# maria-korosteleva/Garment-Pattern-Estimation

Measured on AMD Instinct MI355X. Metric: garments/sec (fwd+bwd) at N=2048 pts, batch 32 per GPU, higher is better.
Workload: dtype f16x3 (fp16 MFMA x3 per product, fp32 accumulate); 1 GPU; BASELINE cfg 2 (cfg 3 per GPU): GarmentFullPattern3D, EdgeConv encoder + LSTM decoders, N=2048, batch 32/GPU, k=16; fp32 storage, fp32-grade arithmetic: edge-GEMM products as 3 fp16 MFMAs on tensor-normalised two-term splits, fp32 accumulate (parity-grade: the exact mode's test bars); global_batch=32, parallelism=dp1, math_mode=f16x3, loss_epoch=0, reserved_cus=0, launch=eager (one Python call per launch), side_stream=True, step=fwd + ComposedPatternLoss + bwd + fused Adam (flat arena)

## Files before the change

garment-pattern-estimation_amd/_lib.py:

```python
import ctypes
import os
import re

import torch

_HERE = os.path.dirname(os.path.abspath(__file__))
LIB_PATH = os.environ.get('GPE_HIP_LIB') or os.path.join(_HERE, 'libgpe_hip.so')
HEADER_PATH = os.path.join(os.path.dirname(_HERE), 'include', 'gpe_hip.h')
EXT_HEADER_PATH = os.path.join(os.path.dirname(_HERE), 'include', 'gpe_hip_ext.h')
HEADERS = (HEADER_PATH, EXT_HEADER_PATH)
FIT_HEADER_PATH = os.path.join(os.path.dirname(_HERE), 'include', 'gpe_hip_fit.h')
FEATURE_HEADERS = (FIT_HEADER_PATH,)
EVAL_HEADER_PATH = os.path.join(os.path.dirname(_HERE), 'include', 'gpe_hip_eval.h')
EVAL_HEADERS = (EVAL_HEADER_PATH,)
PLACE_HEADER_PATH = os.path.join(os.path.dirname(_HERE), 'include', 'gpe_hip_place.h')
PLACE_HEADERS = (PLACE_HEADER_PATH,)
FRAMEWORK_HEADER_PATH = os.path.join(os.path.dirname(_HERE), 'include', 'gpe_hip_framework.h')
FRAMEWORK_HEADERS = (FRAMEWORK_HEADER_PATH,)

_CT = {'p': ctypes.c_void_p, 'i': ctypes.c_int, 'l': ctypes.c_long, 'f': ctypes.c_float, 'd': ctypes.c_double}


def _code(ctype):
    t = ctype.strip()
    if '*' in t:
        return 'p'
    t = t.replace('const', '').strip()
    return {'int': 'i', 'long': 'l', 'float': 'f', 'double': 'd'}[t]


def parse_header(path=HEADER_PATH):
    src = open(path).read()
    src = re.sub(r'/\*.*?\*/', ' ', src, flags=re.S)
    src = re.sub(r'//[^\n]*', ' ', src)
    sigs = {}
    for m in re.finditer(r'\b(int|long)\s+(gpe_\w+)\s*\(([^)]*)\)\s*;', src):
        res, name, args = m.group(1), m.group(2), m.group(3).strip()
        codes = []
        if args and args != 'void':
            for a in args.split(','):
                a = a.strip()
                ctype = a[:a.rfind(' ')] if '*' not in a else a[:a.rfind('*') + 1]
                codes.append(_code(ctype))
        sigs[name] = (_code(res), codes)
    unbound = sorted(set(re.findall(r'\b(gpe_\w+)\s*\(', src)) - set(sigs))
    if unbound:
        raise ValueError('%s: cannot bind the declaration of %s (only functions returning int or long are parsed)'
                         % (path, ', '.join(unbound)))
    return sigs


_lib = None


def lib():
    global _lib
    if _lib is None:
        if not os.path.exists(LIB_PATH):
            raise RuntimeError(
                'libgpe_hip.so not built: run `python -c "import __graft_entry__ as g; g.build()"` '
                '(hipcc --offload-arch=gfx950).  There is no CPU fallback for the product path.')
        l = ctypes.CDLL(LIB_PATH)
        for header in HEADERS + FEATURE_HEADERS + EVAL_HEADERS + PLACE_HEADERS + FRAMEWORK_HEADERS:
            for name, (res, args) in parse_header(header).items():
                fn = getattr(l, name)
                fn.restype = _CT[res]
                fn.argtypes = [_CT[a] for a in args]
        _lib = l
        env = os.environ.get('GPE_MATH')
        if env:
            set_math(env)
        dbg = os.environ.get('GPE_DEBUG_SET')
        if dbg:
            l.gpe_debug_set(int(dbg, 0))
    return _lib


MATH_MODES = {'f32': 0, 'bf16x3': 1, 'mixed': 2, 'bf16x6': 3, 'f16x3': 4}


def set_math(mode):
    if mode not in MATH_MODES:
        raise ValueError('unknown math mode %r (choose from %s)' % (mode, sorted(MATH_MODES)))
    prev = lib().gpe_math_set(MATH_MODES[mode])
    if prev < 0:
        raise RuntimeError('gpe_math_set failed with code %d' % prev)
    return {v: k for k, v in MATH_MODES.items()}[prev]


def set_f16x3_min_rows(rows):
    prev = lib().gpe_f16x3_min_rows_set(int(rows))
    if prev < 0:
        raise RuntimeError('gpe_f16x3_min_rows_set failed with code %d' % prev)
    return prev


def set_reserved_cus(n):
    prev = lib().gpe_reserve_cus_set(int(n))
    if prev < 0:
        raise ValueError('reserved CUs must lie in 0 .. 192')
    return prev


def get_reserved_cus():
    n = lib().gpe_reserve_cus_set(0)
    lib().gpe_reserve_cus_set(n)
    return n


def get_math():
    return {v: k for k, v in MATH_MODES.items()}[lib().gpe_math_get()]


def _conv(a):
    if a is None:
        return None
    if isinstance(a, torch.Tensor):
        return a.data_ptr()
    return a


TIMING = None


_raw_stream = getattr(torch._C, '_cuda_getCurrentRawStream', None)
_cur_device = getattr(torch._C, '_cuda_getDevice', None) or torch.cuda.current_device
_FN = {}


def call(name, *args):
    fn = _FN.get(name)
    if fn is None:
        fn = _FN[name] = getattr(lib(), name)
    cur = _cur_device()
    for a in args:
        if isinstance(a, torch.Tensor):
            if not a.is_cuda or a.device.index != cur:
                raise RuntimeError('%s: tensor on %s but the current device is cuda:%d — wrap the call in '
                                   'torch.cuda.device(...) (one process per GPU is the supported layout)'
                                   % (name, a.device, cur))
            break
    if TIMING is not None or _raw_stream is None:
        stream = torch.cuda.current_stream()
        handle = stream.cuda_stream
    else:
        handle = _raw_stream(cur)
# ... 14 lines not shown
```

garment-pattern-estimation_amd/_opbase.py:

```python
import torch

from . import _lib as L
from . import streams


F32 = torch.float32
F64 = torch.float64


def _dev_check(t):
    if not t.is_cuda:
        raise RuntimeError('gpe ops need tensors on the MI355X (got a %s tensor); there is no CPU path' % t.device)
    if t.dtype != F32:
        raise RuntimeError('gpe ops are fp32 (got %s)' % t.dtype)


def _rows2d(t):
    assert t.dim() == 2 and (t.shape[1] == 1 or t.stride(1) == 1), (t.shape, t.stride())
    return (t, t.stride(0), 0, 0)


def _rows3d(t):
    assert t.dim() == 3 and (t.shape[2] == 1 or t.stride(2) == 1), (t.shape, t.stride())
    return (t, t.stride(0), t.stride(1), t.shape[1])


def round_up(a, b):
    return (a + b - 1) // b * b


_WS = {}


def _workspace(nbytes, device):
    key = streams.stream_key(device)
    buf = _WS.get(key)
    if buf is None or buf.numel() < nbytes:
        buf = torch.empty(max(int(nbytes), 1 << 20), device=torch.device('cuda', key[0]), dtype=torch.uint8)
        _WS[key] = buf
    return buf


_EDGE_WS_BYTES = {}


def edge_workspace(B, N, k, ldmax, device):
    key = (B, N, k, ldmax)
    n = _EDGE_WS_BYTES.get(key)
    if n is None:
        n = L.query('gpe_edge_ws_bytes', B, N, k, ldmax)
        if n < 0:
            raise RuntimeError('gpe_edge_ws_bytes failed with code %d' % n)
        _EDGE_WS_BYTES[key] = n
    return _workspace(n, device), n


def f16x3_words(n, rows, device):
    if L.get_math() != 'f16x3' or rows < L.query('gpe_f16x3_min_rows'):
        return None
    return torch.zeros(n, device=device, dtype=torch.int32)


def _word(words, i):
    return None if words is None else words[i:i + 1]


_TICKETS = {}


def _ticket(device):
    key = streams.stream_key(device)
    t = _TICKETS.get(key)
    if t is None:
        t = _TICKETS[key] = torch.zeros(1, device=torch.device('cuda', key[0]), dtype=torch.int32)
    return t


def _stitch_ldw(H):
    nb = (H + 15) // 16
    nb = 4 if nb <= 4 else 8 if nb <= 8 else 13 if nb <= 13 else 16
    return nb * 16 if (nb * 16) % 32 == 16 else nb * 16 + 16


def _view_strides(ol):
    assert ol.dim() == 4 and ol.stride(3) == 1, (ol.shape, ol.stride())
    return ol.stride(0), ol.stride(1), ol.stride(2)


def _row_stride(t, P):
    assert t.dim() == 3 and t.stride(2) == 1 and t.stride(0) == P * t.stride(1), (t.shape, t.stride())
    return t.stride(1)


def _int_tensor(t, shape, name, dev):
    if (not torch.is_tensor(t) or tuple(t.shape) != shape or t.is_floating_point() or t.is_complex() or t.dtype == torch.bool
            or t.device != dev):
        raise ValueError('%s must be an integer %s tensor on the device of edges3d' % (name, list(shape)))


def _int32(t, lo, hi):
    t = t.detach()
    if t.dtype != torch.int32:
        t = t.to(torch.int64).clamp(lo, hi).to(torch.int32)
    return t.contiguous()
```

garment-pattern-estimation_amd/build.py:

```python
import concurrent.futures
import os
import subprocess
import sys

HERE = os.path.dirname(os.path.abspath(__file__))
CSRC = os.path.join(HERE, 'csrc')
OUT = os.path.join(HERE, 'libgpe_hip.so')
HIPCC = os.environ.get('HIPCC', '/opt/rocm/bin/hipcc')
FLAGS = ['--offload-arch=gfx950', '-O3', '-std=c++17', '-fPIC', '-Wall', '-Wno-unused-function',
         '-Wno-unused-variable', '-Wno-unused-but-set-variable']
EXTRA_FLAGS = {'gpe_edgegemm_sr_dense.hip': ['-mllvm', '-amdgpu-sched-strategy=max-ilp'],
               'gpe_redgemm.hip': ['-mllvm', '-amdgpu-sched-strategy=max-memory-clause'],
               'gpe_knn.hip': ['-mllvm', '-amdgpu-sched-strategy=max-ilp'],
               'gpe_knn_ft.hip': (['-DKNN_FT_TIMING'] if os.environ.get('KNN_FT_TIMING') else []) + os.environ.get('KNN_FT_FLAGS', '').split(),
               'gpe_edgegemm_x6.hip': ['-mllvm', '-amdgpu-sched-strategy=max-memory-clause'],
               'gpe_edgegemm_h3.hip': ['-mllvm', '-amdgpu-sched-strategy=max-ilp'],
               'gpe_edgegemm_w8_f3.hip': ['-mllvm', '-amdgpu-sched-strategy=max-ilp'],
               'gpe_edgegemm_w8_b3.hip': ['-mllvm', '-amdgpu-sched-strategy=max-ilp']}


def _sources():
    return sorted(f for f in os.listdir(CSRC) if f.endswith('.hip'))


def _stale(obj, src):
    if not os.path.exists(obj):
        return True
    t = os.path.getmtime(obj)
    inc = os.path.join(os.path.dirname(HERE), 'include')
    deps = [os.path.join(CSRC, src), os.path.abspath(__file__)]
    deps += [os.path.join(inc, h) for h in ('gpe_hip.h', 'gpe_hip_ext.h', 'gpe_hip_fit.h', 'gpe_hip_eval.h', 'gpe_hip_place.h',
                                              'gpe_hip_framework.h')]
    deps += [os.path.join(CSRC, h) for h in os.listdir(CSRC) if h.endswith('.h')]
    return any(os.path.getmtime(d) > t for d in deps)


COMPILED, REUSED = [], []


def _compile(src):
    obj = os.path.join(CSRC, src[:-4] + '.o')
    if not _stale(obj, src):
        REUSED.append(src)
    else:
        COMPILED.append(src)
        cmd = [HIPCC] + FLAGS + EXTRA_FLAGS.get(src, []) + ['-c', os.path.join(CSRC, src), '-o', obj]
        r = subprocess.run(cmd, capture_output=True, text=True)
        if r.returncode != 0:
            raise RuntimeError('hipcc failed on %s:\n%s' % (src, r.stderr[-6000:]))
        if r.stderr.strip():
            sys.stderr.write(r.stderr[-3000:])
    return obj


def build(force=False, verbose=True):
    force = force or os.environ.get('GPE_FORCE_BUILD') == '1'
    del COMPILED[:], REUSED[:]
    srcs = _sources()
    if force:
        for s in srcs:
            o = os.path.join(CSRC, s[:-4] + '.o')
            if os.path.exists(o):
                os.remove(o)
    with concurrent.futures.ThreadPoolExecutor(max_workers=min(8, len(srcs))) as ex:
        objs = list(ex.map(_compile, srcs))
    if (not os.path.exists(OUT)) or any(os.path.getmtime(o) > os.path.getmtime(OUT) for o in objs):
        cmd = [HIPCC, '--offload-arch=gfx950', '-shared', '-fPIC', '-o', OUT] + objs
        r = subprocess.run(cmd, capture_output=True, text=True)
        if r.returncode != 0:
            raise RuntimeError('link failed:\n' + r.stderr[-4000:])
        if verbose:
            print('built', OUT)
    if verbose:
        print('build: compiled %d source(s) %s; reused %d up-to-date object(s) %s (force=%s; GPE_FORCE_BUILD=1 or '
              'build(force=True) recompiles everything)' % (len(COMPILED), COMPILED, len(REUSED), REUSED, force))
    return OUT


if __name__ == '__main__':
    build(force='--force' in sys.argv)
```

garment-pattern-estimation_amd/csrc/gpe_common.h:

```cpp
#pragma once
#include <cstdlib>
#include <hip/hip_runtime.h>
#include <stdint.h>
#include "../../include/gpe_hip.h"
#include "../../include/gpe_hip_ext.h"
#include "../../include/gpe_hip_fit.h"
#include "../../include/gpe_hip_eval.h"
#include "../../include/gpe_hip_place.h"
#include "../../include/gpe_hip_framework.h"

#define GPE_OK 0
#define GPE_EINVAL (-22)
#define GPE_ELAUNCH (-5)

#define GPE_CHECK_LAUNCH()                                   \
    do {                                                     \
        hipError_t e_ = hipGetLastError();                   \
        if (e_ != hipSuccess) return GPE_ELAUNCH;            \
    } while (0)

typedef float f32x4 __attribute__((ext_vector_type(4)));

static inline bool gpe_overlap(const void* p, size_t n, const void* q, size_t m)
{
    if (!p || !q || !n || !m) return false;
    const uintptr_t a = (uintptr_t)p, b = (uintptr_t)q;
    return a < b + m && b < a + n;
}

static inline const char* gpe_dbg_env_str(const char* name)
{
    static const int on = getenv("GPE_DEBUG") ? atoi(getenv("GPE_DEBUG")) : 0;
    return on ? getenv(name) : nullptr;
}
static inline int gpe_dbg_env(const char* name, int dflt)
{
    const char* e = gpe_dbg_env_str(name);
    return e ? atoi(e) : dflt;
}

static inline int gpe_cdiv(long a, long b) { return (int)((a + b - 1) / b); }
static inline int gpe_round_up(int a, int b) { return (a + b - 1) / b * b; }

struct GpeRows {
    const float* base;
    long stride_outer;
    long stride_inner;
    int inner;
};

__device__ __forceinline__ const float* gpe_row_ptr(const GpeRows& a, long r)
{
    if (a.inner <= 0) return a.base + r * a.stride_outer;
    long o = r / a.inner;
    long i = r - o * a.inner;
    return a.base + o * a.stride_outer + i * a.stride_inner;
}

__device__ __forceinline__ bool gpe_aligned16(const void* p) { return (((uintptr_t)p) & 15) == 0; }

__device__ __forceinline__ unsigned gpe_udiv(unsigned n, unsigned d, double rcp)
{
    unsigned q = (unsigned)__double2uint_rz((double)n * rcp);
    const unsigned up = ((unsigned long long)(q + 1) * d <= n) ? 1u : 0u;
    const unsigned dn = ((unsigned long long)q * d > n) ? 1u : 0u;
    return q + up - dn;
}

#define GPE_ENSURE_MAX_LDS_N(fn, bytes_)                                                                         \
    do {                                                                                                         \
        static unsigned long long done_ = 0;                                                                     \
        int dev_ = 0;                                                                                            \
        if (hipGetDevice(&dev_) != hipSuccess) return GPE_ELAUNCH;                                               \
        const unsigned long long bit_ = 1ull << (dev_ & 63);                                                     \
        if (!(done_ & bit_)) {                                                                                   \
            if (hipFuncSetAttribute(reinterpret_cast<const void*>(fn), hipFuncAttributeMaxDynamicSharedMemorySize, \
                                    (bytes_)) != hipSuccess)                                                     \
                return GPE_ELAUNCH;                                                                              \
            done_ |= bit_;                                                                                       \
        }                                                                                                        \
    } while (0)

#define GPE_ENSURE_MAX_LDS(fn) GPE_ENSURE_MAX_LDS_N(fn, 160 * 1024)

int gpe_num_cus();
int gpe_math_rowgemm();
int gpe_math_redgemm();
#define GPE_WS_DUMMY_BYTES (64 * 512 * 4)
#define GPE_WS_H3_PARTS 1024
#define GPE_WS_H3_BYTES (((2 + 2 * GPE_WS_H3_PARTS) * 4 + 255) & ~255)
struct GpeEdgeWs { float* dummy; unsigned* h3; char* pseudo; size_t pseudo_bytes; };
static inline GpeEdgeWs gpe_edge_ws(void* ws, long bytes)
// ... 90 lines not shown
```

garment-pattern-estimation_amd/csrc/gpe_device.h:

```cpp
#pragma once
#include "gpe_common.h"
#include <math.h>

typedef _Float16 gpe_f16x2 __attribute__((ext_vector_type(2)));
typedef _Float16 gpe_f16x8 __attribute__((ext_vector_type(8)));
typedef __bf16 gpe_bf16x2 __attribute__((ext_vector_type(2)));
typedef __bf16 gpe_bf16x8 __attribute__((ext_vector_type(8)));
typedef float gpe_f32x2 __attribute__((ext_vector_type(2)));
typedef unsigned gpe_u32x2 __attribute__((ext_vector_type(2)));
typedef unsigned gpe_u32x4 __attribute__((ext_vector_type(4)));

__device__ __forceinline__ float gpe_sigmoid(float x) { return 1.f / (1.f + expf(-x)); }

__device__ __forceinline__ void gpe_split2_f16(float a, float b, unsigned& h, unsigned& l)
{
    const gpe_f32x2 v = {a, b};
    const gpe_f16x2 hh = __builtin_convertvector(v, gpe_f16x2);
    const gpe_f32x2 r = v - __builtin_convertvector(hh, gpe_f32x2);
    h = __builtin_bit_cast(unsigned, hh);
    l = __builtin_bit_cast(unsigned, __builtin_convertvector(r, gpe_f16x2));
}
__device__ __forceinline__ void gpe_split2_f16(float a, float b, float s, unsigned& h, unsigned& l) { gpe_split2_f16(a * s, b * s, h, l); }

__device__ __forceinline__ unsigned gpe_cvt2_bf16(float a, float b)
{
    const gpe_f32x2 v = {a, b};
    return __builtin_bit_cast(unsigned, __builtin_convertvector(v, gpe_bf16x2));
}
__device__ __forceinline__ void gpe_split2_bf16(float a, float b, unsigned& h, unsigned& l)
{
    h = gpe_cvt2_bf16(a, b);
    l = gpe_cvt2_bf16(a - __uint_as_float(h << 16), b - __uint_as_float(h & 0xffff0000u));
}

#define GPE_STATE_SA 4096.f
#define GPE_STATE_INV_SA (1.f / 4096.f)

__device__ __forceinline__ gpe_u32x4 gpe_philox4x32(unsigned c0, unsigned c1, unsigned c2, unsigned c3, unsigned k0, unsigned k1)
{
#pragma unroll
    for (int r = 0; r < 10; ++r) {
        const unsigned hi0 = __umulhi(0xD2511F53u, c0), lo0 = 0xD2511F53u * c0;
        const unsigned hi1 = __umulhi(0xCD9E8D57u, c2), lo1 = 0xCD9E8D57u * c2;
        c0 = hi1 ^ c1 ^ k0; c1 = lo1; c2 = hi0 ^ c3 ^ k1; c3 = lo0;
        k0 += 0x9E3779B9u; k1 += 0xBB67AE85u;
    }
    return gpe_u32x4{c0, c1, c2, c3};
}
struct gpe_rng {
    unsigned k0, k1, d0, d1, b8;
    __device__ __forceinline__ gpe_u32x4 operator()(int kind, unsigned item, unsigned attempt = 0) const
    {
        return gpe_philox4x32(item | ((unsigned)kind << 28), attempt | b8, d0, d1, k0, k1);
    }
};

#define GPE_SPIN_LIMIT (1u << 23)

__device__ __forceinline__ unsigned gpe_flag_load(const unsigned* flag)
{
    return __hip_atomic_load(flag, __ATOMIC_RELAXED, __HIP_MEMORY_SCOPE_AGENT);
}
__device__ __forceinline__ unsigned gpe_flag_poll(const unsigned* flag) { return __builtin_amdgcn_readfirstlane(gpe_flag_load(flag)); }
__device__ __forceinline__ void gpe_flag_wait(const unsigned* flag, unsigned need)
{
    unsigned spins = 0;
    while (gpe_flag_poll(flag) < need) {
        __builtin_amdgcn_s_sleep(1);
        if (++spins > GPE_SPIN_LIMIT) __builtin_trap();
    }
    asm volatile("" ::: "memory");
}
__device__ __forceinline__ void gpe_drain_stores() { asm volatile("s_waitcnt vmcnt(0)" ::: "memory"); }
__device__ __forceinline__ unsigned gpe_flag_ticket(unsigned* flag)
{
    return __hip_atomic_fetch_add(flag, 1u, __ATOMIC_RELAXED, __HIP_MEMORY_SCOPE_AGENT);
}
__device__ __forceinline__ void gpe_flag_arrive_wave(unsigned* flag)
{
    gpe_drain_stores();
    if ((threadIdx.x & 63) == 0) gpe_flag_ticket(flag);
}
__device__ __forceinline__ void gpe_flag_arrive_wg(unsigned* flag, unsigned long long* stamp = nullptr)
{
    gpe_drain_stores();
    if (stamp && threadIdx.x == 0) *stamp = wall_clock64();
    __syncthreads();
// ... 50 lines not shown
```

garment-pattern-estimation_amd/csrc/gpe_edgegemm_h3.hip:

```cpp
#include "gpe_edgegemm_split_kernel.h"

#define H3_PQ_BLOCKS GPE_WS_H3_PARTS

__global__ __launch_bounds__(256) void gpe_h3_absmax_kernel(const float* __restrict__ x, long rows, int cols4, long ld,
                                                            unsigned* __restrict__ out)
{
    const long total = rows * cols4;
    unsigned m = 0u;
    for (long t = (long)blockIdx.x * blockDim.x + threadIdx.x; t < total; t += (long)gridDim.x * blockDim.x) {
        const long r = t / cols4;
        const int q = (int)(t - r * cols4);
        const float4 v = ld4(x + r * ld + 4 * q);
        const unsigned a = __float_as_uint(v.x) & 0x7fffffffu, b = __float_as_uint(v.y) & 0x7fffffffu;
        const unsigned c = __float_as_uint(v.z) & 0x7fffffffu, d = __float_as_uint(v.w) & 0x7fffffffu;
        const unsigned ab = a > b ? a : b, cd = c > d ? c : d;
        const unsigned e = ab > cd ? ab : cd;
        m = m > e ? m : e;
    }
#pragma unroll
    for (int o = 32; o > 0; o >>= 1) {
        const unsigned t = (unsigned)__shfl_xor((int)m, o);
        m = m > t ? m : t;
    }
    __shared__ unsigned red[4];
    if ((threadIdx.x & 63) == 0) red[threadIdx.x >> 6] = m;
    __syncthreads();
    if (threadIdx.x == 0) {
        const unsigned a = red[0] > red[1] ? red[0] : red[1], b = red[2] > red[3] ? red[2] : red[3];
        const unsigned r = a > b ? a : b;
        if (r) atomicMax(out, r);
    }
}

__global__ __launch_bounds__(256) void gpe_h3_pqmax_kernel(const float* __restrict__ pq, long rows, int H, long ld,
                                                           float* __restrict__ part )
{
    const int lane = threadIdx.x & 63, wave = threadIdx.x >> 6;
    const int h4 = H >> 2;
    float mp = -INFINITY, mq = -INFINITY;
    const long stride = (long)gridDim.x * 4;
    for (long r = (long)blockIdx.x * 4 + wave; r < rows; r += 2 * stride) {
        const float* row0 = pq + r * ld;
        const bool two = r + stride < rows;
        const float* row1 = pq + (two ? r + stride : r) * ld;
        for (int q = lane; q < 2 * h4; q += 64) {
            const float4 v0 = ld4(row0 + 4 * q), v1 = ld4(row1 + 4 * q);
            const float m = fmaxf(fmaxf(fmaxf(v0.x, v0.y), fmaxf(v0.z, v0.w)), fmaxf(fmaxf(v1.x, v1.y), fmaxf(v1.z, v1.w)));
            if (q < h4) mp = fmaxf(mp, m); else mq = fmaxf(mq, m);
        }
    }
#pragma unroll
    for (int o = 32; o > 0; o >>= 1) { mp = fmaxf(mp, __shfl_xor(mp, o)); mq = fmaxf(mq, __shfl_xor(mq, o)); }
    __shared__ float red[8];
    if (lane == 0) { red[2 * wave] = mp; red[2 * wave + 1] = mq; }
    __syncthreads();
    if (threadIdx.x == 0) {
        part[2 * blockIdx.x] = fmaxf(fmaxf(red[0], red[2]), fmaxf(red[4], red[6]));
        part[2 * blockIdx.x + 1] = fmaxf(fmaxf(red[1], red[3]), fmaxf(red[5], red[7]));
    }
}

__global__ __launch_bounds__(1024) void gpe_h3_wmax_kernel(const float* __restrict__ w, long n, unsigned* __restrict__ slots,
                                                           unsigned* __restrict__ clear_word)
{
    __shared__ unsigned red[16];
    unsigned m = 0u;
    for (long t = threadIdx.x; t < n; t += 1024) {
        const unsigned a = __float_as_uint(w[t]) & 0x7fffffffu;
        m = m > a ? m : a;
    }
#pragma unroll
    for (int o = 32; o > 0; o >>= 1) {
        const unsigned t = (unsigned)__shfl_xor((int)m, o);
        m = m > t ? m : t;
    }
    if ((threadIdx.x & 63) == 0) red[threadIdx.x >> 6] = m;
    __syncthreads();
    if (threadIdx.x == 0) {
        for (int i = 1; i < 16; ++i) m = m > red[i] ? m : red[i];
        slots[1] = m;
        slots[0] = 0u;
        if (clear_word) clear_word[0] = 0u;
    }
}

__global__ __launch_bounds__(256) void gpe_h3_pqfinish_kernel(const float* __restrict__ part, int nblk, unsigned* __restrict__ slots)
{
    float mp = -INFINITY, mq = -INFINITY;
    for (int b = threadIdx.x; b < nblk; b += 256) { mp = fmaxf(mp, part[2 * b]); mq = fmaxf(mq, part[2 * b + 1]); }
#pragma unroll
    for (int o = 32; o > 0; o >>= 1) { mp = fmaxf(mp, __shfl_xor(mp, o)); mq = fmaxf(mq, __shfl_xor(mq, o)); }
    __shared__ float red[8];
    if ((threadIdx.x & 63) == 0) { red[2 * (threadIdx.x >> 6)] = mp; red[2 * (threadIdx.x >> 6) + 1] = mq; }
    __syncthreads();
    if (threadIdx.x == 0) {
        mp = fmaxf(fmaxf(red[0], red[2]), fmaxf(red[4], red[6]));
        mq = fmaxf(fmaxf(red[1], red[3]), fmaxf(red[5], red[7]));
        float b = (mp + mq) * 1.000001f;
        if (!(b > 0.f)) b = (b != b) ? b : 0.f;
        slots[0] = __float_as_uint(b) & 0x7fffffffu;
    }
}

int gpe_h3_pq_passes(unsigned* out, float* part, const float* pq, long rows, int H, long ld, hipStream_t s)
{
    if (!out || !part || (H & 3)) return GPE_EINVAL;
    int gx = (int)((rows + 3) / 4);
    if (gx > H3_PQ_BLOCKS) gx = H3_PQ_BLOCKS;
    hipLaunchKernelGGL(gpe_h3_pqmax_kernel, dim3(gx), dim3(256), 0, s, pq, rows, H, ld, part);
    GPE_CHECK_LAUNCH();
    hipLaunchKernelGGL(gpe_h3_pqfinish_kernel, dim3(1), dim3(256), 0, s, part, gx, out);
    GPE_CHECK_LAUNCH();
    return GPE_OK;
}
static int h3_absmax_pass(unsigned* out, const float* x, long rows, int cols4, long ld, hipStream_t s)
{
    int gx = (int)((rows * cols4 + 255) / 256);
    const int cap = gpe_num_cus() * 8;
    if (gx > cap) gx = cap;
    hipLaunchKernelGGL(gpe_h3_absmax_kernel, dim3(gx), dim3(256), 0, s, x, rows, cols4, ld, out);
    GPE_CHECK_LAUNCH();
    return GPE_OK;
}
int gpe_h3_absmax(unsigned* out, const float* x, long rows, int cols, long ld, hipStream_t s)
{
    if (!out || !x) return GPE_EINVAL;
    if (hipMemsetAsync(out, 0, sizeof(unsigned), s) != hipSuccess) return GPE_ELAUNCH;
    const int cols4 = (cols + 3) >> 2;
    if (rows * cols4 <= 0) return GPE_OK;
    return h3_absmax_pass(out, x, rows, cols4, ld, s);
}

int gpe_edge_f16x3_scales(RgParams& p, long npts, int amode, int emode, int KCH, hipStream_t s)
{
    unsigned* slots = p.ws.h3;
    const bool tracks = emode == E_EDGE_FWD || emode == E_BWD_INPLACE;
    const bool reuse = (p.dbg & 128) != 0;
    const long wn = (long)16 * KCH * p.Npad;
    const bool w_ready = p.w_ready && p.user_amax_a;
    if (!reuse && !w_ready) {
        hipLaunchKernelGGL(gpe_h3_wmax_kernel, dim3(1), dim3(1024), 0, s, p.wp, wn, slots, tracks ? p.user_amax_out : nullptr);
        GPE_CHECK_LAUNCH();
    }
    p.h3_amax_a = (p.user_amax_a && !reuse) ? p.user_amax_a : slots;
    if (!p.user_amax_a && !reuse) {
        const int rc = amode == A_DENSE ? h3_absmax_pass(slots, p.a.base, p.M, (p.K + 3) >> 2, (long)p.a.stride_outer, s)
                                        : gpe_h3_pq_passes(slots, reinterpret_cast<float*>(slots + 2), p.pq, npts, p.H, (long)p.ldpq, s);
        if (rc != GPE_OK) return rc;
    }
    p.h3_amax_w = slots + 1;
// ... 11 lines not shown
```

garment-pattern-estimation_amd/csrc/gpe_knn.hip:

```cpp
#include "gpe_device.h"
#include "gpe_knn_plan.h"
#include <math.h>
#include <stdint.h>
#include <stdlib.h>

#define KNN_CCH 32
#define KNN_LD 36
#define KNN_LDD 68

__device__ __forceinline__ float knn_readlane_f(float v, int l)
{
    return __int_as_float(__builtin_amdgcn_readlane(__float_as_int(v), l));
}

__device__ __forceinline__ float knn_sub(float a, float b)
{
    float d;
    asm("v_sub_f32 %0, %1, %2" : "=v"(d) : "v"(a), "v"(b));
    return d;
}
__device__ __forceinline__ float knn_sqacc(float d, float acc)
{
    asm("v_fma_f32 %0, %1, %1, %0" : "+v"(acc) : "v"(d));
    return acc;
// ... 584 lines not shown
        asm volatile("s_waitcnt lgkmcnt(0)" ::: "memory");

        const int cand = c0 + lane;
#pragma unroll
        for (int i = 0; i < 16; ++i) {
            if (!((qm >> i) & 1u)) continue;
            const float d = dW[i * KNN_LDD + lane];
            float ldv = ld_[i];
            int liv = li_[i];
            const float t = knn_select_mf(c0 == c_first, d, lane, cand, K2, kk, knn_readlane_f(m2e_of, i),
                                          knn_readlane_f(thrq, i), mW, ldv, liv);
            ld_[i] = ldv; li_[i] = liv;
            thrq = ((lane & 15) == i) ? t : thrq;
            __builtin_amdgcn_sched_barrier(0);
        }
    }
#pragma unroll
    for (int i = 0; i < 16; ++i) {
        const int q = q0 + 16 * wave + i;
        if (q < N && lane < K2)
            part[(((size_t)b * N + q) * nsplit + piece) * K2 + lane] =
                ((unsigned long long)(unsigned)__float_as_int(ld_[i]) << 32) | (unsigned)li_[i];
    }
}

#define KNN_H3_CCH 64
#define KNN_H3_PITCH 160

__global__ __launch_bounds__(256) void gpe_knn_planes_kernel(const float* __restrict__ x, long rows, int C, int ldx, int CP,
                                                             _Float16* __restrict__ pl, float* __restrict__ isc,
                                                             const int* __restrict__ order, int N)
{
    const int lane = threadIdx.x & 63;
    const long r0 = ((long)blockIdx.x * 4 + (threadIdx.x >> 6)) * KNN_NORM_ROWS;
    if (r0 >= rows) return;
    const long last = rows - 1;
    long src[KNN_NORM_ROWS];
#pragma unroll
    for (int u = 0; u < KNN_NORM_ROWS; ++u) {
        const long r = (r0 + u < last) ? r0 + u : last;
        src[u] = order ? (r / N) * N + order[r] : r;
    }
    float m[KNN_NORM_ROWS];
#pragma unroll
    for (int u = 0; u < KNN_NORM_ROWS; ++u) m[u] = 0.f;
    for (int c0 = 0; c0 < C; c0 += 64) {
        const int c = c0 + lane;
        const int cc = (c < C) ? c : 0;
        float v[KNN_NORM_ROWS];
#pragma unroll
        for (int u = 0; u < KNN_NORM_ROWS; ++u) v[u] = x[src[u] * ldx + cc];
#pragma unroll
        for (int u = 0; u < KNN_NORM_ROWS; ++u) m[u] = (c < C) ? fmaxf(m[u], fabsf(v[u])) : m[u];
    }
    float sc[KNN_NORM_ROWS];
#pragma unroll
    for (int u = 0; u < KNN_NORM_ROWS; ++u) {
        float t = m[u];
#pragma unroll
        for (int o = 32; o > 0; o >>= 1) t = fmaxf(t, __int_as_float(__builtin_amdgcn_ds_bpermute((lane ^ o) << 2, __float_as_int(t))));
        float s_, inv_;
        gpe_h3_scale_of(__float_as_uint(t), s_, inv_);
        sc[u] = s_;
        if (lane == 0 && r0 + u <= last) isc[r0 + u] = inv_;
    }
    for (int c0 = 0; c0 < CP; c0 += 64) {
        const int c = c0 + lane;
        if (c >= CP) break;
        const int cc = (c < C) ? c : 0;
        float v[KNN_NORM_ROWS];
#pragma unroll
        for (int u = 0; u < KNN_NORM_ROWS; ++u) v[u] = x[src[u] * ldx + cc];
#pragma unroll
        for (int u = 0; u < KNN_NORM_ROWS; ++u) {
            if (r0 + u <= last) {
                const float xs = (c < C) ? v[u] * sc[u] : 0.f;
                const _Float16 h = (_Float16)xs;
                const _Float16 l = (_Float16)(xs - (float)h);
                _Float16* row = pl + (r0 + u) * 2 * (long)CP;
                row[c] = h;
                row[CP + c] = l;
            }
        }
    }
}

template <int NBMAX>
__global__ __launch_bounds__(256, 2) void gpe_knn_h3_kernel(const _Float16* __restrict__ pl, const float* __restrict__ isc, int N,
                                                            int CP, int kk, int K2, const float* __restrict__ norms,
                                                            const int* __restrict__ cmax, float ce, int B, int tiles, int pin,
                                                            int nsplit, unsigned long long* __restrict__ part, int probe,
                                                            const int* __restrict__ ord)
{
    const int rot = ord != nullptr;
    extern __shared__ __align__(16) float smem[];
    constexpr int PLANE_B = KNN_TC * KNN_H3_PITCH;
    constexpr int BUF_B = 2 * PLANE_B;
    char* const cB = reinterpret_cast<char*>(smem);
    float* const dS = reinterpret_cast<float*>(cB + 2 * BUF_B);
    unsigned long long* const mS = reinterpret_cast<unsigned long long*>(dS + 4 * 16 * KNN_LDD);
    float* const npS = reinterpret_cast<float*>(mS + 4 * 64);
    float* const isS = npS + 2 * KNN_TC;

    const int tid = threadIdx.x;
    const int lane = tid & 63;
    const int wave = __builtin_amdgcn_readfirstlane(tid >> 6);
    int b, item;
    const int ipc = tiles * nsplit;
    if (pin) {
        const int xcd = blockIdx.x & (GPE_NXCD - 1), slot = blockIdx.x >> 3;
        const int jc = slot / ipc;
        b = xcd + GPE_NXCD * jc;
        item = slot - jc * ipc;
        if (b >= B) return;
    } else {
        b = blockIdx.x / ipc;
        item = blockIdx.x - b * ipc;
    }
    const int qt = item / nsplit, piece = item - qt * nsplit;
    const int q0 = qt * KNN_TQ;
    const int tps = (tiles + nsplit - 1) / nsplit;
    const int c_first = piece * tps * KNN_TC;
    const int c_stop = ((piece + 1) * tps * KNN_TC < N) ? (piece + 1) * tps * KNN_TC : N;
    const _Float16* cloud = pl + (size_t)b * N * 2 * CP;
    const float* cnorm = norms + (size_t)b * N;
    const float* cisc = isc + (size_t)b * N;
    const int* cord = ord ? ord + (size_t)b * N : nullptr;
    auto pt = [&](int r) -> int { return cord ? cord[r] : r; };
    float* const dW = dS + wave * 16 * KNN_LDD;
    unsigned long long* const mW = mS + wave * 64;

    float ld_[16];
    int li_[16];
#pragma unroll
    for (int i = 0; i < 16; ++i) { ld_[i] = INFINITY; li_[i] = -1; }
    float thrq = INFINITY;

    const int j = lane & 15, g = lane >> 4;
    const int myq = (q0 + 16 * wave + j < N) ? q0 + 16 * wave + j : N - 1;
    const float nq = cnorm[pt(myq)];
    const float fq = -2.f * cisc[myq];
    const float cm = __int_as_float(cmax[b]);
    float m2e_of;
    {
        const int qi = (q0 + 16 * wave + (lane & 15) < N) ? q0 + 16 * wave + (lane & 15) : N - 1;
        m2e_of = 2.02f * ce * (cnorm[pt(qi)] + cm);
    }
    const int NB = CP >> 5;
    gpe_u32x4 qh[NBMAX], ql[NBMAX];
    {
        const _Float16* qrow = cloud + (size_t)myq * 2 * CP;
#pragma unroll
        for (int blk = 0; blk < NBMAX; ++blk) {
            const int bb = (blk < NB) ? blk : 0;
            qh[blk] = *reinterpret_cast<const gpe_u32x4*>(qrow + 32 * bb + 8 * g);
            ql[blk] = *reinterpret_cast<const gpe_u32x4*>(qrow + CP + 32 * bb + 8 * g);
        }
    }
    const int nchunk = (CP + KNN_H3_CCH - 1) / KNN_H3_CCH;
    gpe_u32x4 pre[4];
    float pre_n = 0.f, pre_s = 0.f;
    int pre_first = 0, pre_tp = 0;
    const int ntile_p = (c_stop - c_first + KNN_TC - 1) / KNN_TC;
    int v_start = 0;
    if (rot && ntile_p > 0) {
        v_start = qt - 1 - c_first / KNN_TC;
// ... 290 lines not shown

__global__ __launch_bounds__(256) void gpe_knn_rerank2_kernel(const float* __restrict__ x, long nq_total, int N, int C, int ldx, int k,
                                                              const unsigned long long* __restrict__ part,
                                                              const float* __restrict__ norms, const int* __restrict__ cmax,
                                                              float ce, int32_t* __restrict__ idx, int32_t* __restrict__ idx_glob)
{
    __shared__ unsigned long long strip[4][64];
    const int lane = threadIdx.x & 63;
    const int wave = __builtin_amdgcn_readfirstlane(threadIdx.x >> 6);
    const long q0 = ((long)blockIdx.x * 4 + wave) * 2;
    if (q0 >= nq_total) return;
    unsigned long long* const mW = strip[wave];
    const int h = lane >> 5, l = lane & 31;
    const bool two = q0 + 1 < nq_total;
    const long q = (h && two) ? q0 + 1 : q0;
    unsigned long long key = part[q * 64 + l];
    const unsigned long long hi32 = part[q * 64 + 32 + l];
    const unsigned long long v_lo = __ballot(key != ~0ull), v_hi = __ballot(hi32 != ~0ull);
    const bool packable = (v_hi == 0ull) && k <= 32;
    if (!packable) {
        knn_rerank_query(x, q0, N, C, ldx, k, 64, 1, part, norms, cmax, ce, idx, idx_glob, 1, mW);
        if (two) knn_rerank_query(x, q0 + 1, N, C, ldx, k, 64, 1, part, norms, cmax, ce, idx, idx_glob, 1, mW);
        return;
    }
    const int nv = __builtin_popcount((unsigned)(v_lo >> (32 * h)));
    const int nvmax = max(__builtin_popcount((unsigned)v_lo), __builtin_popcount((unsigned)(v_lo >> 32)));
    const int base = 32 * h;
    {
        int rank = 0;
        const int klo = (int)(unsigned)key, khi = (int)(unsigned)(key >> 32);
        for (int s2 = 0; s2 < nvmax; ++s2) {
            const unsigned long long kn = ((unsigned long long)(unsigned)__shfl(khi, base + s2) << 32) | (unsigned)__shfl(klo, base + s2);
            rank += (s2 < nv && (kn < key || (kn == key && s2 < l))) ? 1 : 0;
        }
        if (l >= nv) rank = l;
        mW[base + rank] = key;
        asm volatile("s_waitcnt lgkmcnt(0)" ::: "memory");
        key = mW[lane];
        asm volatile("s_waitcnt lgkmcnt(0)" ::: "memory");
    }
    const float da = __int_as_float((int)(key >> 32));
    const int id = (int)(unsigned)key;
    const int b = (int)(q / N);
    const float* cloud = x + (size_t)b * N * ldx;
    const float* qrow = x + q * ldx;
    const bool vec4 = (ldx % 4 == 0) && ((uintptr_t)x % 16 == 0);
    const float m2e = 2.02f * ce * (norms[q] + __int_as_float(cmax[b]));
    const float T = __shfl(da, base + k - 1) + m2e;
    const unsigned long long below = __ballot(l < nv && da <= T);
    const int m = __builtin_popcount((unsigned)(below >> base));
    const int mmax = max(__builtin_popcount((unsigned)below), __builtin_popcount((unsigned)(below >> 32)));
    const bool in_s = l < m;
    const float dnext = __shfl(da, (lane + 1) & 63);
    const bool near_next = (l + 1 < m) && (dnext - da <= m2e);
    const unsigned long long nn = __ballot(near_next);
    const bool near_prev = (l > 0) && ((nn >> (lane - 1)) & 1ull);
    const bool flagged = in_s && (near_next || near_prev);
    const unsigned long long fl = __ballot(flagged);
    int newpos = l;
    if (fl) {
        const unsigned long long starts = __ballot(in_s && !near_prev);
        const unsigned long long le = ((lane == 63) ? ~0ull : ((1ull << (lane + 1)) - 1ull)) & (0xffffffffull << base);
        const int start = 63 - __builtin_clzll((starts & le) | (1ull << base));
        float dex = da;
        if (flagged) dex = knn_exact_chain(qrow, cloud + (size_t)id * ldx, C, vec4);
        int r = 0;
        for (int s2 = 0; s2 < mmax; ++s2) {
            const float dj = __shfl(dex, base + s2);
            const int ij = __shfl(id, base + s2);
            const int sj = __shfl(start, base + s2);
            r += (s2 < m && sj == start && (dj < dex || (dj == dex && ij < id))) ? 1 : 0;
        }
        if (flagged) newpos = (start - base) + r;
    }
    if (in_s && newpos < k && (h == 0 || two)) {
        idx[q * k + newpos] = id;
        if (idx_glob) idx_glob[q * k + newpos] = b * N + id;
    }
}

int gpe_knn_launch_prologue(const GpeKnnCall& c, const GpeKnnPlan& p)
{
    const long nq = (long)c.B * c.N;
    if (p.identity) {
        hipLaunchKernelGGL(gpe_knn_identity_order_kernel, dim3((unsigned)gpe_cdiv(nq, 256)), dim3(256), 0, c.stream, c.order_out, nq, c.N);
        GPE_CHECK_LAUNCH();
    }
    if (p.norms) {
        hipLaunchKernelGGL(gpe_knn_norms_kernel, dim3((unsigned)gpe_cdiv(nq, 4 * KNN_NORM_ROWS)), dim3(256), 0, c.stream, c.x, nq, c.N, c.C,
                           c.ldx, p.norms, p.cmax);
        GPE_CHECK_LAUNCH();
        hipLaunchKernelGGL(gpe_knn_cmax_kernel, dim3(c.B), dim3(256), 0, c.stream, p.norms, c.N, p.cmax);
        GPE_CHECK_LAUNCH();
    }
    if (p.planes) {
        hipLaunchKernelGGL(gpe_knn_planes_kernel, dim3((unsigned)gpe_cdiv(nq, 4 * KNN_NORM_ROWS)), dim3(256), 0, c.stream, c.x, nq, c.C,
                           c.ldx, p.CP, p.planes, p.iscale, p.order, c.N);
        GPE_CHECK_LAUNCH();
    }
    return GPE_OK;
}

int gpe_knn_launch_lists(const GpeKnnCall& c, const GpeKnnPlan& p)
{
    const size_t lds = (size_t)2 * 2 * KNN_TC * KNN_H3_PITCH + (size_t)4 * 16 * KNN_LDD * sizeof(float) +
                       4 * 64 * sizeof(unsigned long long) + 4 * KNN_TC * sizeof(float);
    auto go = [&](auto kernel) {
        hipLaunchKernelGGL(kernel, dim3((unsigned)p.nblocks), dim3(256), lds, c.stream, p.planes, p.iscale, c.N, p.CP, c.k, p.K2, p.norms,
                           p.cmax, p.ce, c.B, p.tiles, p.pin, p.nsplit, p.part, p.probe, p.order);
    };
    if (p.NB <= 2) go(gpe_knn_h3_kernel<2>);
    else if (p.NB <= 5) go(gpe_knn_h3_kernel<5>);
    else go(gpe_knn_h3_kernel<8>);
    GPE_CHECK_LAUNCH();
    return GPE_OK;
}

int gpe_knn_launch_f32filter(const GpeKnnCall& c, const GpeKnnPlan& p)
{
    const size_t lds = ((size_t)2 * KNN_TQ * KNN_MF_LD + 4 * 16 * KNN_LDD) * sizeof(float) + 4 * 64 * sizeof(unsigned long long) +
                       KNN_TC * sizeof(float);
    auto go = [&](auto kernel) {
        hipLaunchKernelGGL(kernel, dim3((unsigned)p.nblocks), dim3(256), lds, c.stream, c.x, c.N, c.C, c.ldx, c.k, p.K2, p.norms, p.cmax,
                           p.ce, c.B, p.tiles, p.pin, p.nsplit, p.part, p.probe);
    };
    if (p.vec == 4) go(gpe_knn_mfma_kernel<4>);
    else if (p.vec == 2) go(gpe_knn_mfma_kernel<2>);
    else go(gpe_knn_mfma_kernel<1>);
    GPE_CHECK_LAUNCH();
    return GPE_OK;
}

int gpe_knn_launch_recheck(const GpeKnnCall& c, const GpeKnnPlan& p)
{
    const long nq = (long)c.B * c.N;
    if (p.rerank2)
        hipLaunchKernelGGL(gpe_knn_rerank2_kernel, dim3((unsigned)gpe_cdiv(nq, 8)), dim3(256), 0, c.stream, c.x, nq, c.N, c.C, c.ldx, c.k,
                           p.part, p.norms, p.cmax, p.ce, c.idx, c.idx_glob);
    else
        hipLaunchKernelGGL(gpe_knn_rerank_kernel, dim3((unsigned)gpe_cdiv(nq, 4)), dim3(256), 0, c.stream, c.x, nq, c.N, c.C, c.ldx, c.k,
                           p.K2, p.nsplit, p.part, p.norms, p.cmax, p.ce, c.idx, c.idx_glob, p.unsorted);
    GPE_CHECK_LAUNCH();
    return GPE_OK;
}
```

garment-pattern-estimation_amd/csrc/gpe_knn_plan.h:

```cpp
#pragma once
#include "gpe_common.h"

#define KNN_TQ 64
#define KNN_TC 64
#define KNN_MF_MINC 16
#define KNN_H3_MAXC 256
#define KNN_FT_NBMAX 5
#define KNN_FT_MAXK 32
#define KNN_FT_CAP 64
#define K3_MINN 128
#define K3_MAXN 8192
#ifndef K3_QW
#define K3_QW 4
#endif
#define KNN_FILTER_MAXK 48

struct GpeKnnSwitches {
    int PROBE;
    int PIN;
    int VEC;
    int SPLIT;
    int EXACT;
    int F32FILTER;
    int SORTED;
    int NOORDER;
    int FT;
    int RR2;
};
const GpeKnnSwitches& gpe_knn_switches();

struct GpeKnnCall {
    const float* x; int B, N, C, ldx, k;
    int32_t* idx; int32_t* idx_glob;
    const int32_t* order_in; int32_t* order_out;
    void* ws; long ws_bytes;
    hipStream_t stream;
};

static_assert(sizeof(float4) + 8 * sizeof(float) <= 64 * sizeof(unsigned long long), "sorted cloud + tile boxes must fit the list region");
struct GpeKnnWs {
    size_t lists_bytes;
    size_t norms, cmax, planes, iscale;
    size_t tb, sorted_bytes;
    size_t need_f32;
    size_t need_h3;
    size_t total;
};
static inline size_t gpe_knn_up256(size_t b) { return (b + 255) & ~(size_t)255; }
static inline GpeKnnWs gpe_knn_ws_layout(int B, int N, int C)
{
    GpeKnnWs w;
    const size_t nq = (size_t)B * N;
    const size_t norm_bytes = gpe_knn_up256(nq * sizeof(float)), cmax_bytes = gpe_knn_up256((size_t)B * sizeof(int));
    const size_t CP = ((size_t)C + 31) & ~(size_t)31;
    const size_t pl_bytes = gpe_knn_up256(nq * 2 * CP * sizeof(_Float16));
    w.lists_bytes = nq * 64 * sizeof(unsigned long long);
    w.norms = w.lists_bytes;
    w.cmax = w.norms + norm_bytes;
    w.planes = w.cmax + cmax_bytes;
    w.iscale = w.planes + pl_bytes;
    w.tb = nq * sizeof(float4);
    w.sorted_bytes = w.tb + (size_t)B * gpe_cdiv(N, 64) * 8 * sizeof(float);
    w.need_f32 = w.planes + 256;
    w.need_h3 = w.need_f32 + pl_bytes + norm_bytes;
    w.total = ((C >= KNN_MF_MINC && C <= KNN_H3_MAXC) ? w.need_h3 : w.need_f32) + 256;
    return w;
}
static inline size_t gpe_knn_split_bytes(int B, int N, int nsplit, int k) { return (size_t)B * N * nsplit * k * sizeof(unsigned long long); }

enum GpeKnnPath {
    GPE_KNN_NOTHING,
    GPE_KNN_SORTED3,
    GPE_KNN_ALLPAIRS,
    GPE_KNN_SCAN,
    GPE_KNN_LISTS,
    GPE_KNN_F32FILTER
};
struct GpeKnnPlan {
    GpeKnnPath path; int rc;
    bool identity;
    int pin, tiles, nsplit, vec;
    long nblocks;
    int probe; bool smallc;
    int K2, CP, NB; float ce;
    bool wide; int qtiles;
    bool rerank2; int unsorted;
    const int32_t* order;
    unsigned long long* part;
    float* norms; int* cmax; _Float16* planes; float* iscale;
    float4* xs; float* tb;
};

static inline int gpe_knn_k2(int k, int N)
{
    int K2 = (2 * k < 32) ? 2 * k : 32;
    if (K2 < k + 8) K2 = k + 8;
    if (K2 > 64) K2 = 64;
    if (K2 > N) K2 = N;
    return K2;
}
static inline bool gpe_knn_valid(const GpeKnnCall& c)
{
    return c.x && c.idx && c.B >= 0 && c.N > 0 && c.C > 0 && c.ldx >= c.C && c.k > 0 && c.k <= 64 && c.k <= c.N &&
           (long)c.B * c.N * c.k < (1L << 31);
}
static inline bool gpe_knn_ws_holds(const GpeKnnCall& c, size_t bytes) { return c.ws && !(((uintptr_t)c.ws) & 15) && (size_t)c.ws_bytes >= bytes; }
static inline long gpe_knn_tile_blocks(int pin, int B, int tiles) { return pin ? (long)GPE_NXCD * gpe_cdiv(B, GPE_NXCD) * tiles : (long)B * tiles; }
static inline GpeKnnPlan gpe_knn_refuse(GpeKnnPlan p, int rc) { p.path = GPE_KNN_NOTHING; p.rc = rc; p.identity = false; return p; }

static inline GpeKnnPlan gpe_knn_plan_allpairs(GpeKnnPlan p, const GpeKnnCall& c, int usable_cus, const GpeKnnSwitches& sw, bool with_ws)
{
    p.path = GPE_KNN_ALLPAIRS;
    p.nsplit = 1;
    if (p.pin) {
        const double table = (double)c.N * c.ldx * sizeof(float), l2_budget = 3.2 * 1024 * 1024;
        const int resident = 4 * usable_cus / GPE_NXCD;
        for (;;) {
            const double clouds = (double)resident / ((double)p.tiles * p.nsplit);
            if (table * (clouds > 1.0 ? clouds : 1.0) <= l2_budget) break;
            if (clouds <= 1.0) break;
            if (p.nsplit >= 4 || 2 * p.nsplit * c.k > 64 || 2 * p.nsplit > p.tiles) break;
            p.nsplit *= 2;
        }
    }
    if (sw.SPLIT > 0 && sw.SPLIT * c.k <= 64 && sw.SPLIT <= p.tiles) p.nsplit = sw.SPLIT;
    if (p.nsplit > 1) {
        if (with_ws && gpe_knn_ws_holds(c, gpe_knn_split_bytes(c.B, c.N, p.nsplit, c.k))) p.part = (unsigned long long*)c.ws;
        else p.nsplit = 1;
    }
    p.nblocks = gpe_knn_tile_blocks(p.pin, c.B, p.tiles) * p.nsplit;
    if (p.nblocks >= (1L << 31)) return gpe_knn_refuse(p, GPE_EINVAL);
    const uintptr_t xa = (uintptr_t)c.x;
    p.vec = (c.C % 4 == 0 && c.ldx % 4 == 0 && xa % 16 == 0) ? 4 : (c.C % 2 == 0 && c.ldx % 2 == 0 && xa % 8 == 0) ? 2 : 1;
    if (sw.VEC > 0 && sw.VEC < p.vec) p.vec = sw.VEC;
    p.probe = sw.PROBE;
    p.smallc = !p.probe && p.vec == 1 && c.C <= 4;
    return p;
}

static inline GpeKnnPlan gpe_knn_plan(const GpeKnnCall& c, int usable_cus, const GpeKnnSwitches& sw)
{
    GpeKnnPlan p = {};
    p.path = GPE_KNN_NOTHING;
    p.rc = GPE_OK;
    if (!gpe_knn_valid(c)) return gpe_knn_refuse(p, GPE_EINVAL);
    if (c.B == 0) return p;
    p.tiles = gpe_cdiv(c.N, KNN_TQ);
    p.pin = (sw.PIN >= 0) ? (sw.PIN && c.B >= GPE_NXCD) : (gpe_pin_clouds(c.B) ? 1 : 0);
    p.nsplit = 1;
    const GpeKnnWs w = gpe_knn_ws_layout(c.B, c.N, c.C);
    if (c.C < KNN_MF_MINC || c.k > KNN_FILTER_MAXK || sw.EXACT) {
        if (c.C == 3 && sw.SORTED != 0 && c.N >= K3_MINN && c.N <= K3_MAXN && gpe_knn_ws_holds(c, w.sorted_bytes) &&
            (long)c.B * gpe_cdiv(c.N, 4 * K3_QW) < (1L << 31)) {
            p.path = GPE_KNN_SORTED3;
            p.tiles = gpe_cdiv(c.N, 64);
            p.qtiles = gpe_cdiv(c.N, 4 * K3_QW);
            p.nblocks = (long)c.B * p.qtiles;
            p.xs = reinterpret_cast<float4*>(c.ws);
            p.tb = reinterpret_cast<float*>(reinterpret_cast<char*>(c.ws) + w.tb);
            return p;
        }
        p.identity = c.order_out != nullptr;
        return gpe_knn_plan_allpairs(p, c, usable_cus, sw, true);
    }
    p.identity = c.order_out != nullptr;
    p.K2 = gpe_knn_k2(c.k, c.N);
    if (sw.SPLIT > 0 && sw.SPLIT * p.K2 <= 64 && sw.SPLIT <= p.tiles) p.nsplit = sw.SPLIT;
    bool h3 = !sw.F32FILTER && c.C <= KNN_H3_MAXC;
    if (h3 && (!c.ws || (size_t)c.ws_bytes < w.need_h3)) h3 = false;
    if (!gpe_knn_ws_holds(c, h3 ? w.need_h3 : w.need_f32)) return gpe_knn_plan_allpairs(p, c, usable_cus, sw, false);
    char* const scratch = (char*)c.ws;
    p.part = (unsigned long long*)scratch;
    p.norms = (float*)(scratch + w.norms);
    p.cmax = (int*)(scratch + w.cmax);
    p.CP = (c.C + 31) & ~31;
    p.NB = p.CP >> 5;
    p.ce = (6.f * c.C + (h3 ? 32.f : 16.f)) * 5.9604645e-8f;
    p.probe = sw.PROBE;
    p.nblocks = gpe_knn_tile_blocks(p.pin, c.B, p.tiles) * p.nsplit;
    if (p.nblocks >= (1L << 31)) return gpe_knn_refuse(p, GPE_EINVAL);
    if (!h3) {
        p.path = GPE_KNN_F32FILTER;
        const uintptr_t xa = (uintptr_t)c.x;
        p.vec = (c.ldx % 4 == 0 && xa % 16 == 0 && ((c.C + 3) & ~3) <= c.ldx) ? 4
              : (c.ldx % 2 == 0 && xa % 8 == 0 && ((c.C + 1) & ~1) <= c.ldx) ? 2 : 1;
        if (sw.VEC > 0 && sw.VEC < p.vec) p.vec = sw.VEC;
        return p;
    }
    p.planes = (_Float16*)(scratch + w.planes);
    p.iscale = (float*)(scratch + w.iscale);
    p.order = sw.NOORDER ? nullptr : c.order_in;
    if (sw.FT && p.NB <= KNN_FT_NBMAX && c.k <= KNN_FT_MAXK && p.nsplit == 1) {
        p.path = GPE_KNN_SCAN;
        p.wide = sw.FT == 8 || (sw.FT != 4 && (long)c.B * gpe_cdiv(c.N, 128) >= usable_cus);
        p.qtiles = gpe_cdiv(c.N, p.wide ? 128 : 64);
        p.nblocks = gpe_knn_tile_blocks(p.pin, c.B, p.qtiles);
        p.rerank2 = sw.RR2 != 0;
        p.unsorted = 1;
        return p;
    }
    p.path = GPE_KNN_LISTS;
    return p;
}

int gpe_knn_launch_prologue(const GpeKnnCall& c, const GpeKnnPlan& p);
int gpe_knn_launch_allpairs(const GpeKnnCall& c, const GpeKnnPlan& p);
int gpe_knn_launch_lists(const GpeKnnCall& c, const GpeKnnPlan& p);
int gpe_knn_launch_f32filter(const GpeKnnCall& c, const GpeKnnPlan& p);
int gpe_knn_launch_recheck(const GpeKnnCall& c, const GpeKnnPlan& p);
int gpe_knn_launch_sorted(const GpeKnnCall& c, const GpeKnnPlan& p);
int gpe_knn_launch_scan(const GpeKnnCall& c, const GpeKnnPlan& p);
```

garment-pattern-estimation_amd/csrc/gpe_knn_search.hip:

```cpp
#include "gpe_knn_plan.h"

const GpeKnnSwitches& gpe_knn_switches()
{
    static const GpeKnnSwitches sw = {gpe_dbg_env("GPE_KNN_PROBE", 0),  gpe_dbg_env("GPE_KNN_PIN", -1),  gpe_dbg_env("GPE_KNN_VEC", 0),
                                      gpe_dbg_env("GPE_KNN_SPLIT", 0),  gpe_dbg_env("GPE_KNN_EXACT", 0), gpe_dbg_env("GPE_KNN_F32FILTER", 0),
                                      gpe_dbg_env("GPE_KNN_SORTED", 1), gpe_dbg_env("GPE_KNN_NOORDER", 0), gpe_dbg_env("GPE_KNN_FT", 1),
                                      gpe_dbg_env("GPE_KNN_RR2", 1)};
    return sw;
}

extern "C" long gpe_knn_ws_bytes(int B, int N, int C, int k)
{
    if (B < 0 || N <= 0 || C <= 0 || k <= 0 || k > 64) return GPE_EINVAL;
    return (long)gpe_knn_ws_layout(B, N, C).total;
}

extern "C" int gpe_knn(const float* x, int B, int N, int C, int ldx, int k, int32_t* idx, int32_t* idx_glob, const int32_t* order_in,
                       int32_t* order_out, void* ws, long ws_bytes, void* stream)
{
    const GpeKnnCall c = {x, B, N, C, ldx, k, idx, idx_glob, order_in, order_out, ws, ws_bytes, (hipStream_t)stream};
    if (!gpe_knn_valid(c)) return GPE_EINVAL;
    const GpeKnnPlan p = gpe_knn_plan(c, B ? gpe_num_cus() : 0, gpe_knn_switches());
    if (p.path == GPE_KNN_NOTHING) return p.rc;
    int rc = gpe_knn_launch_prologue(c, p);
    if (rc != GPE_OK) return rc;
    switch (p.path) {
    case GPE_KNN_SORTED3: return gpe_knn_launch_sorted(c, p);
    case GPE_KNN_ALLPAIRS: return gpe_knn_launch_allpairs(c, p);
    case GPE_KNN_SCAN: rc = gpe_knn_launch_scan(c, p); break;
    case GPE_KNN_LISTS: rc = gpe_knn_launch_lists(c, p); break;
    default: rc = gpe_knn_launch_f32filter(c, p); break;
    }
    return rc != GPE_OK ? rc : gpe_knn_launch_recheck(c, p);
}
```

garment-pattern-estimation_amd/csrc/gpe_pointwise.hip:

```cpp
#include "gpe_device.h"
#include <math.h>

__device__ __forceinline__ float4 pw_ld4(const float* p) { return *reinterpret_cast<const float4*>(p); }
__device__ __forceinline__ void pw_st4(float* p, float4 v) { *reinterpret_cast<float4*>(p) = v; }

static int gpe_pack_kpad(int K)
{
    const int k16 = gpe_round_up(K, 16);
    return (k16 > 96 && k16 < 160) ? 160 : (k16 > 160 && k16 < 208) ? 208 : k16;
}
extern "C" long gpe_packed_size(int N, int K) { return (long)gpe_round_up(N, 16) * gpe_pack_kpad(K); }

__global__ void gpe_pack_kernel(const float* __restrict__ w, int ldw, int N, int K, int transpose,
                                const float* __restrict__ col_scale, float* __restrict__ wp, int Npad, long total)
{
    const long e = (long)blockIdx.x * blockDim.x + threadIdx.x;
    if (e >= total) return;
    const int t = (int)(e & 3);
    const long r = e >> 2;
    const int n = (int)(r % Npad);
    const long kq = r / Npad;
    const int k = (int)(kq * 4 + t);
    float v = 0.f;
    if (n < N && k < K) {
// ... 515 lines not shown
        s += __shfl_xor(s, o);
        q += __shfl_xor(q, o);
    }
    if (sub == 0) { red[wave][0][ch] = s; red[wave][1][ch] = q; }
    __syncthreads();
    if (wave != 0 || sub != 0 || c >= C) return;
    s = 0; q = 0;
    for (int w_ = 0; w_ < BNF_WAVES; ++w_) { s += red[w_][0][ch]; q += red[w_][1][ch]; }
    const double mean = s / count;
    double var = q / count - mean * mean;
    if (var < 0) var = 0;
    const double rstd = 1.0 / sqrt(var + (double)eps);
    const float sc = (float)((double)gamma[c] * rstd);
    stats[c] = (float)mean;
    stats[C + c] = (float)rstd;
    stats[2 * C + c] = sc;
    stats[3 * C + c] = (float)((double)beta[c] - mean * (double)sc);
    if (running_mean) {
        const double unbiased = (count > 1) ? var * count / (count - 1) : var;
        running_mean[c] = (float)((1.0 - momentum) * running_mean[c] + momentum * mean);
        running_var[c] = (float)((1.0 - momentum) * running_var[c] + momentum * unbiased);
    }
}

extern "C" int gpe_bn_finalize(const double* part, int nblk, int C, double count, const float* gamma,
                               const float* beta, float eps, float momentum, float* running_mean,
                               float* running_var, int64_t* num_batches, float* stats_out, void* stream)
{
    if (!part || !gamma || !beta || !stats_out || nblk <= 0 || C <= 0 || count <= 0) return GPE_EINVAL;
    hipLaunchKernelGGL(gpe_bn_finalize_kernel, dim3(gpe_cdiv(C, BNF_CPW)), dim3(64 * BNF_WAVES), 0, (hipStream_t)stream, part, nblk,
                       C, count, gamma, beta, eps, momentum, running_mean, running_var, num_batches, stats_out);
    GPE_CHECK_LAUNCH();
    return GPE_OK;
}

__global__ void gpe_bn_from_running_kernel(const float* rm, const float* rv, int C, const float* gamma,
                                           const float* beta, float eps, float* stats)
{
    const int c = blockIdx.x * blockDim.x + threadIdx.x;
    if (c >= C) return;
    const double rstd = 1.0 / sqrt((double)rv[c] + (double)eps);
    const float sc = (float)((double)gamma[c] * rstd);
    stats[c] = rm[c];
    stats[C + c] = (float)rstd;
    stats[2 * C + c] = sc;
    stats[3 * C + c] = (float)((double)beta[c] - (double)rm[c] * (double)sc);
}

extern "C" int gpe_bn_from_running(const float* running_mean, const float* running_var, int C, const float* gamma,
                                   const float* beta, float eps, float* stats_out, void* stream)
{
    if (!running_mean || !running_var || !gamma || !beta || !stats_out || C <= 0) return GPE_EINVAL;
    hipLaunchKernelGGL(gpe_bn_from_running_kernel, dim3(gpe_cdiv(C, 64)), dim3(64), 0, (hipStream_t)stream,
                       running_mean, running_var, C, gamma, beta, eps, stats_out);
    GPE_CHECK_LAUNCH();
    return GPE_OK;
}

__global__ void gpe_edge_finish_kernel(const float* __restrict__ mx, const float* __restrict__ mn, int ldagg,
                                       const float* __restrict__ stats, long rows, int C, float* __restrict__ y,
                                       int ldy)
{
    const long e = (long)blockIdx.x * blockDim.x + threadIdx.x;
    if (e >= rows * C) return;
    const long r = e / C;
    const int c = (int)(e - r * C);
    const float s = stats[2 * C + c], t = stats[3 * C + c];
    const float v = (s >= 0.f) ? mx[r * ldagg + c] : mn[r * ldagg + c];
    y[r * ldy + c] = s * v + t;
}

extern "C" int gpe_edge_finish(const float* mx, const float* mn, int ldagg, const float* stats, long rows, int C,
                               float* y, int ldy, void* stream)
{
    if (!mx || !mn || !stats || !y || rows < 0 || C <= 0 || ldagg < C || ldy < C) return GPE_EINVAL;
    if (rows == 0) return GPE_OK;
    hipLaunchKernelGGL(gpe_edge_finish_kernel, dim3(gpe_cdiv(rows * C, 256)), dim3(256), 0, (hipStream_t)stream, mx,
                       mn, ldagg, stats, rows, C, y, ldy);
    GPE_CHECK_LAUNCH();
    return GPE_OK;
}

#define PS_BLOCKS 512
__global__ __launch_bounds__(256) void gpe_point_sums_kernel(const float* __restrict__ g, int ldg,
                                                             const float* __restrict__ mx,
                                                             const float* __restrict__ mn, int ldagg,
                                                             const float* __restrict__ stats, long rows, int C,
                                                             double* __restrict__ part, unsigned* __restrict__ amax_sg)
{
    const int c = blockIdx.y * 256 + threadIdx.x;
    double s1 = 0, s2 = 0;
    float gm = 0.f, sabs = 0.f;
    if (c < C) {
        const float mean = stats[c], rstd = stats[C + c], s = stats[2 * C + c];
        const float* sp = (s >= 0.f) ? mx : mn;
        const long st = gridDim.x;
        long r = blockIdx.x;
        for (; r + 7 * st < rows; r += 8 * st) {
            float gv[8], sv[8];
#pragma unroll
            for (int u = 0; u < 8; ++u) { gv[u] = g[(r + u * st) * ldg + c]; sv[u] = sp[(r + u * st) * ldagg + c]; }
#pragma unroll
            for (int u = 0; u < 8; ++u) {
                s1 += (double)gv[u];
                s2 += (double)gv[u] * (double)((sv[u] - mean) * rstd);
                gm = fmaxf(gm, fabsf(gv[u]));
            }
        }
        for (; r < rows; r += st) {
            const float gv = g[r * ldg + c];
            const float sel = sp[r * ldagg + c];
            s1 += (double)gv;
            s2 += (double)gv * (double)((sel - mean) * rstd);
            gm = fmaxf(gm, fabsf(gv));
        }
        part[(size_t)blockIdx.x * 2 * C + c] = s1;
        part[(size_t)blockIdx.x * 2 * C + C + c] = s2;
        sabs = fabsf(s);
    }
    if (amax_sg) {
        float m = gm * sabs;
#pragma unroll
        for (int o = 32; o > 0; o >>= 1) m = fmaxf(m, __shfl_xor(m, o));
        if ((threadIdx.x & 63) == 0) atomicMax(amax_sg, __float_as_uint(m * 1.0000002f));
    }
}

extern "C" int gpe_point_sums_blocks(void) { return PS_BLOCKS; }

extern "C" int gpe_edge_bwd_point_sums(const float* g, int ldg, const float* mx, const float* mn, int ldagg,
                                       const float* stats, long rows, int C, double* part, uint32_t* amax_sg, void* stream)
{
    if (!g || !mx || !mn || !stats || !part || rows <= 0 || C <= 0) return GPE_EINVAL;
    if (amax_sg && hipMemsetAsync(amax_sg, 0, sizeof(uint32_t), (hipStream_t)stream) != hipSuccess) return GPE_ELAUNCH;
    hipLaunchKernelGGL(gpe_point_sums_kernel, dim3(PS_BLOCKS, gpe_cdiv(C, 256)), dim3(256), 0, (hipStream_t)stream, g, ldg, mx, mn,
                       ldagg, stats, rows, C, part, amax_sg);
    GPE_CHECK_LAUNCH();
    return GPE_OK;
}

#define BNC_WAVES 16
__global__ __launch_bounds__(64 * BNC_WAVES) void gpe_bn_bwd_coef_kernel(const double* __restrict__ part, int nblk,
                                                                        const float* __restrict__ stats, int C, double count,
                                                                        float* __restrict__ coef, float* dgamma, float* dbeta)
{
    __shared__ double red[BNC_WAVES][2][64];
    const int lane = threadIdx.x & 63, wave = threadIdx.x >> 6;
    const int c = blockIdx.x * 64 + lane;
    double s1 = 0, s2 = 0;
    if (c < C) {
        for (int b = wave; b < nblk; b += BNC_WAVES) {
            s1 += part[(size_t)b * 2 * C + c];
            s2 += part[(size_t)b * 2 * C + C + c];
        }
    }
    red[wave][0][lane] = s1;
    red[wave][1][lane] = s2;
    __syncthreads();
    if (wave != 0 || c >= C) return;
    s1 = 0; s2 = 0;
    for (int w_ = 0; w_ < BNC_WAVES; ++w_) { s1 += red[w_][0][lane]; s2 += red[w_][1][lane]; }
    const double mean = stats[c], rstd = stats[C + c], s = stats[2 * C + c];
    const double m1 = s1 / count, m2 = s2 / count;
    const double k2 = s * rstd * m2;
    coef[c] = (float)s;
    coef[C + c] = (float)(s * m1);
    coef[2 * C + c] = (float)k2;
    coef[3 * C + c] = (float)mean;
    if (dgamma) dgamma[c] = (float)s2;
    if (dbeta) dbeta[c] = (float)s1;
}

extern "C" int gpe_bn_bwd_coef(const double* part, int nblk, const float* stats, int C, double count, float* coef,
                               float* dgamma, float* dbeta, void* stream)
{
    if (!part || !stats || !coef || nblk <= 0 || C <= 0 || count <= 0) return GPE_EINVAL;
    hipLaunchKernelGGL(gpe_bn_bwd_coef_kernel, dim3(gpe_cdiv(C, 64)), dim3(64 * BNC_WAVES), 0, (hipStream_t)stream, part, nblk,
                       stats, C, count, coef, dgamma, dbeta);
    GPE_CHECK_LAUNCH();
    return GPE_OK;
}

#define DZ3_RB 8
__global__ __launch_bounds__(256) void gpe_dz3_kernel(float* __restrict__ a3, int lda3, const float* __restrict__ g,
                                                      int ldg, const uint8_t* __restrict__ amx,
                                                      const uint8_t* __restrict__ amn, int ldagg,
                                                      const float* __restrict__ coef, long npts, int k, int F,
                                                      float gscale, unsigned* __restrict__ amax_out)
{
    __shared__ unsigned amax_red[4];
    if (threadIdx.x < 4) amax_red[threadIdx.x] = 0u;
    __syncthreads();
    float amax_run = 0.f;
    const int lane = threadIdx.x & 63;
    const int wave = __builtin_amdgcn_readfirstlane(threadIdx.x >> 6);
    const int c = (blockIdx.y * 64 + lane) << 2;
    if (c >= F) return;
    const bool all_slots = amx == nullptr;
    float cs_[4], c1_[4], k2_[4], mu_[4];
#pragma unroll
    for (int t = 0; t < 4; ++t) {
        const int cc = (c + t < F) ? c + t : c;
        cs_[t] = coef[cc]; c1_[t] = coef[F + cc]; k2_[t] = coef[2 * F + cc]; mu_[t] = coef[3 * F + cc];
    }
    const long nw = (long)gridDim.x * 4;
    for (long i = (long)blockIdx.x * 4 + wave; i < npts; i += nw) {
        uint8_t mxv[4] = {0, 0, 0, 0}, mnv[4] = {0, 0, 0, 0};
        if (!all_slots) {
            const uchar4 smx = *reinterpret_cast<const uchar4*>(amx + i * ldagg + c);
            const uchar4 smn = *reinterpret_cast<const uchar4*>(amn + i * ldagg + c);
            mxv[0] = smx.x; mxv[1] = smx.y; mxv[2] = smx.z; mxv[3] = smx.w;
            mnv[0] = smn.x; mnv[1] = smn.y; mnv[2] = smn.z; mnv[3] = smn.w;
        }
        int sel[4];
        float sg[4];
#pragma unroll
        for (int t = 0; t < 4; ++t) {
            const int cc = (c + t < F) ? c + t : c;
            sel[t] = (cs_[t] >= 0.f) ? mxv[t] : mnv[t];
            sg[t] = cs_[t] * g[i * ldg + cc] * gscale;
        }
        float* base = a3 + i * k * lda3 + c;
        for (int s0 = 0; s0 < k; s0 += DZ3_RB) {
            float4 a[DZ3_RB];
#pragma unroll
            for (int u = 0; u < DZ3_RB; ++u) {
                const int s_ = (s0 + u < k) ? s0 + u : k - 1;
                a[u] = pw_ld4(base + (long)s_ * lda3);
            }
#pragma unroll
            for (int u = 0; u < DZ3_RB; ++u) {
                if (s0 + u < k) {
                    const float av[4] = {a[u].x, a[u].y, a[u].z, a[u].w};
                    float o[4];
#pragma unroll
                    for (int t = 0; t < 4; ++t) {
                        const float hit = (all_slots || sel[t] == s0 + u) ? sg[t] : 0.f;
                        o[t] = (c + t < F && av[t] > 0.f) ? hit - c1_[t] - (av[t] - mu_[t]) * k2_[t] : 0.f;
                    }
                    pw_st4(base + (long)(s0 + u) * lda3, make_float4(o[0], o[1], o[2], o[3]));
                    amax_run = fmaxf(fmaxf(amax_run, fmaxf(fabsf(o[0]), fabsf(o[1]))), fmaxf(fabsf(o[2]), fabsf(o[3])));
                }
            }
        }
    }
    if (amax_out) {
        atomicMax(&amax_red[wave], __float_as_uint(amax_run));
        __syncthreads();
        if (threadIdx.x == 0) {
            const unsigned a = amax_red[0] > amax_red[1] ? amax_red[0] : amax_red[1];
            const unsigned b = amax_red[2] > amax_red[3] ? amax_red[2] : amax_red[3];
            atomicMax(amax_out, a > b ? a : b);
        }
    }
}

static int dz3_launch(float* a3, int lda3, const float* g, int ldg, const uint8_t* amx, const uint8_t* amn, int ldagg,
                      const float* coef, int B, int N, int k, int F, float gscale, unsigned* amax_out, hipStream_t stream)
{
    if (!a3 || !g || !coef || B <= 0 || N <= 0 || k <= 0 || F <= 0 || (lda3 & 3) || lda3 < F) return GPE_EINVAL;
    if (amx && (!amn || (ldagg & 3) || ldagg < F)) return GPE_EINVAL;
    const long E = (long)B * N * k;
    if (E >= (1L << 31)) return GPE_EINVAL;
    const long npts = (long)B * N;
    const int blocks = (int)((npts + 3) / 4 < 4096 ? (npts + 3) / 4 : 4096);
    if (amax_out && hipMemsetAsync(amax_out, 0, sizeof(unsigned), stream) != hipSuccess) return GPE_ELAUNCH;
    hipLaunchKernelGGL(gpe_dz3_kernel, dim3(blocks, gpe_cdiv(F, 256)), dim3(256), 0, stream, a3, lda3, g, ldg, amx, amn,
                       ldagg, coef, npts, k, F, gscale, amax_out);
    GPE_CHECK_LAUNCH();
    return GPE_OK;
}

extern "C" int gpe_edge_dz3(float* a3, int lda3, const float* g, int ldg, const uint8_t* amx, const uint8_t* amn,
                            int ldagg, const float* coef, int B, int N, int k, int F, uint32_t* amax_out, void* stream)
{
    if (!amx || !amn) return GPE_EINVAL;
    return dz3_launch(a3, lda3, g, ldg, amx, amn, ldagg, coef, B, N, k, F, 1.f, amax_out, (hipStream_t)stream);
}

extern "C" int gpe_edge_dz3_all(float* a3, int lda3, const float* g, int ldg, float gscale, const float* coef, int B,
                                int N, int k, int F, uint32_t* amax_out, void* stream)
{
    return dz3_launch(a3, lda3, g, ldg, nullptr, nullptr, 0, coef, B, N, k, F, gscale, amax_out, (hipStream_t)stream);
}

#define BNG_FQ 16
__global__ __launch_bounds__(64 * BNG_FQ) void gpe_bn_bwd_from_G_kernel(
    const float* __restrict__ G, int ldG, const float* __restrict__ db, const float* __restrict__ w, int ldw, int Cn,
    int C, const float* __restrict__ stats, double* __restrict__ sums, float* __restrict__ dw, int lddw)
{
    __shared__ double red[BNG_FQ][2][64];
    const int lane = threadIdx.x & 63, fq = threadIdx.x >> 6;
    const int c = blockIdx.x * 64 + lane;
    double a = 0, b = 0;
    if (c < C) {
        const double s = stats[2 * C + c], t = stats[3 * C + c], mean = stats[c];
        const double beta = t + mean * s;
        double a2[2] = {0, 0}, b2[2] = {0, 0};
        int f = fq;
        for (; f + BNG_FQ < Cn; f += 2 * BNG_FQ) {
#pragma unroll
            for (int u = 0; u < 2; ++u) {
                const int ff = f + BNG_FQ * u;
                const double wf = w[(size_t)ff * ldw + c], gf = G[(size_t)ff * ldG + c], dbf = db[ff];
                a2[u] += wf * dbf;
                b2[u] += wf * gf;
                if (dw) dw[(size_t)ff * lddw + c] = (float)(gf * s + dbf * beta);
            }
        }
        if (f < Cn) {
            const double wf = w[(size_t)f * ldw + c], gf = G[(size_t)f * ldG + c], dbf = db[f];
            a2[0] += wf * dbf;
            b2[0] += wf * gf;
            if (dw) dw[(size_t)f * lddw + c] = (float)(gf * s + dbf * beta);
        }
        a = a2[0] + a2[1];
        b = b2[0] + b2[1];
    }
    red[fq][0][lane] = a;
    red[fq][1][lane] = b;
    __syncthreads();
    if (fq != 0 || c >= C) return;
    a = 0; b = 0;
    for (int q = 0; q < BNG_FQ; ++q) { a += red[q][0][lane]; b += red[q][1][lane]; }
    sums[c] = a;
    sums[C + c] = b * (double)stats[C + c];
}

extern "C" int gpe_bn_bwd_from_G(const float* G, int ldG, const float* db, const float* w_next, int ldw, int Cn,
                                 int C, const float* stats, double* sums, float* dw, int lddw, void* stream)
{
    if (!G || !db || !w_next || !stats || !sums || Cn <= 0 || C <= 0 || ldG < C || ldw < C) return GPE_EINVAL;
    hipLaunchKernelGGL(gpe_bn_bwd_from_G_kernel, dim3(gpe_cdiv(C, 64)), dim3(64 * BNG_FQ), 0, (hipStream_t)stream, G, ldG, db,
                       w_next, ldw, Cn, C, stats, sums, dw, lddw);
    GPE_CHECK_LAUNCH();
    return GPE_OK;
}

template <bool LDS_EDGES>
__global__ __launch_bounds__(1024) void gpe_knn_reverse_kernel(const int32_t* __restrict__ idx, int N, int k,
                                                               int32_t* __restrict__ rev_off,
                                                               int32_t* __restrict__ rev_edge)
{
    extern __shared__ int sm[];
    int* cnt = sm;
    int* off = sm + N;
    __shared__ int wsum[16];
    const int tid = threadIdx.x, b = blockIdx.x;
    const int32_t* id = idx + (size_t)b * N * k;
    int32_t* ro = rev_off + (size_t)b * (N + 1);
    int32_t* const re_g = rev_edge + (size_t)b * N * k;
    int32_t* const re = LDS_EDGES ? reinterpret_cast<int32_t*>(sm + 2 * N + 1) : re_g;
    const int E = N * k;
    for (int i = tid; i < N; i += 1024) cnt[i] = 0;
    __syncthreads();
    for (int e = tid; e < E; e += 1024) atomicAdd(&cnt[id[e]], 1);
    __syncthreads();
    const int per = (N + 1023) / 1024;
    const int beg = tid * per;
    int local = 0;
    for (int i = 0; i < per; ++i) if (beg + i < N) local += cnt[beg + i];
    int x = local;
    const int lane = tid & 63, wv = tid >> 6;
    for (int d = 1; d < 64; d <<= 1) { int y = __shfl_up(x, d); if (lane >= d) x += y; }
    if (lane == 63) wsum[wv] = x;
    __syncthreads();
    if (tid == 0) { int a = 0; for (int w = 0; w < 16; ++w) { int t = wsum[w]; wsum[w] = a; a += t; } }
    __syncthreads();
    int run = x - local + wsum[wv];
    for (int i = 0; i < per; ++i) if (beg + i < N) { off[beg + i] = run; run += cnt[beg + i]; }
    if (tid == 1023) off[N] = E;
    __syncthreads();
    for (int i = tid; i <= N; i += 1024) ro[i] = off[i];
    for (int i = tid; i < N; i += 1024) cnt[i] = 0;
    __syncthreads();
    for (int e = tid; e < E; e += 1024) {
        const int jn = id[e];
        const int pos = atomicAdd(&cnt[jn], 1);
        re[off[jn] + pos] = e;
    }
    __threadfence_block();
    __syncthreads();
    for (int jn = tid; jn < N; jn += 1024) {
        const int a = off[jn], z = off[jn + 1];
        for (int i = a + 1; i < z; ++i) {
            const int v = re[i];
            int h = i - 1;
            while (h >= a && re[h] > v) { re[h + 1] = re[h]; --h; }
            re[h + 1] = v;
        }
    }
    if (LDS_EDGES) {
        __syncthreads();
        for (int e = tid; e < E; e += 1024) re_g[e] = re[e];
    }
}

extern "C" int gpe_knn_reverse(const int32_t* idx, int B, int N, int k, int32_t* rev_off, int32_t* rev_edge,
                               void* stream)
{
    if (!idx || !rev_off || !rev_edge || B <= 0 || N <= 0 || k <= 0) return GPE_EINVAL;
    const size_t lds = (size_t)(2 * N + 1) * sizeof(int);
    if (lds > 150 * 1024) return GPE_EINVAL;
    const size_t lds_e = lds + (size_t)N * k * sizeof(int);
    if (lds_e <= 150 * 1024) {
        GPE_ENSURE_MAX_LDS_N((gpe_knn_reverse_kernel<true>), 150 * 1024);
        hipLaunchKernelGGL(gpe_knn_reverse_kernel<true>, dim3(B), dim3(1024), lds_e, (hipStream_t)stream, idx, N, k, rev_off,
                           rev_edge);
    } else {
        GPE_ENSURE_MAX_LDS_N((gpe_knn_reverse_kernel<false>), 150 * 1024);
        hipLaunchKernelGGL(gpe_knn_reverse_kernel<false>, dim3(B), dim3(1024), lds, (hipStream_t)stream, idx, N, k, rev_off,
                           rev_edge);
    }
    GPE_CHECK_LAUNCH();
    return GPE_OK;
}

// ... 574 lines not shown
```

garment-pattern-estimation_amd/csrc/gpe_redgemm.hip:

```cpp
#include "gpe_device.h"
#include "gpe_redgemm_plan.h"
#include <limits.h>
#include <stdlib.h>

#ifndef RD_B3_PIPE
#define RD_B3_PIPE 0
#endif
#ifndef RD_B3_DBG
#define RD_B3_DBG 0
#endif
#ifndef RD_B3_PRIO
#define RD_B3_PRIO 1
#endif
#ifndef RD_B3_LEFT_CONS
#define RD_B3_LEFT_CONS 0
#endif

__device__ __forceinline__ float4 rd_ld4(const float* p) { return *reinterpret_cast<const float4*>(p); }

__device__ __forceinline__ float4 rd_ld4_guard(const float* p, int nvalid, bool vec)
{
    if (nvalid >= 4 && vec) return rd_ld4(p);
    float4 v = make_float4(0.f, 0.f, 0.f, 0.f);
    if (nvalid > 0) v.x = p[0];
// ... 1024 lines not shown
                        cs[q][c] += uu[c];
#pragma unroll
                        for (int n = 0; n < 4; ++n) acc[q][c][n] = __builtin_fmaf(uu[c], v[j][n], acc[q][c][n]);
                    }
                }
            }
        }
    }
    float* mine = smem + (size_t)wave * p.MgPad * 5;
#pragma unroll
    for (int q = 0; q < QL; ++q) {
        const int c0 = 4 * (lane + 64 * q);
        if (c0 < p.MgPad) {
#pragma unroll
            for (int c = 0; c < 4; ++c) {
#pragma unroll
                for (int n = 0; n < 4; ++n) mine[(c0 + c) * 5 + n] = acc[q][c][n];
                mine[(c0 + c) * 5 + 4] = cs[q][c];
            }
        }
    }
    __syncthreads();
    float* dst = p.part + (size_t)blockIdx.x * p.MgPad * p.NgPad;
    const size_t wstride = (size_t)p.MgPad * 5;
    for (int m = tid; m < p.MgPad; m += 256) {
        const float* s0 = smem + (size_t)m * 5;
#pragma unroll
        for (int n = 0; n < 4; ++n)
            dst[(size_t)m * 4 + n] = (float)(((double)s0[n] + (double)s0[wstride + n]) +
                                             ((double)s0[2 * wstride + n] + (double)s0[3 * wstride + n]));
        if (p.part_cs)
            p.part_cs[(size_t)blockIdx.x * p.MgPad + m] = ((double)s0[4] + (double)s0[wstride + 4]) +
                                                          ((double)s0[2 * wstride + 4] + (double)s0[3 * wstride + 4]);
    }
}

__global__ __launch_bounds__(RD_FIN_E * RD_FIN_Q) void gpe_redgemm_finish(
    const float* __restrict__ part, const double* __restrict__ part_cs, int nblk, int Mg, int Ng, int MgPad, int NgPad,
    float* G, int ldg, float* colsum, int accumulate)
{
    __shared__ double red[RD_FIN_Q][RD_FIN_E];
    const int el = threadIdx.x & (RD_FIN_E - 1), q = threadIdx.x / RD_FIN_E;
    const long total = (long)Mg * Ng;
    const long e = (long)blockIdx.x * RD_FIN_E + el;
    const long g_blocks = (total + RD_FIN_E - 1) / RD_FIN_E;
    const bool is_cs = (long)blockIdx.x >= g_blocks;
    double s0 = 0, s1 = 0;
    if (!is_cs) {
        if (e < total) {
            const int m = (int)(e / Ng), n = (int)(e - (long)m * Ng);
            const size_t stride = (size_t)MgPad * NgPad;
            const float* src = part + (size_t)m * NgPad + n;
            int b = q;
            for (; b + RD_FIN_Q < nblk; b += 2 * RD_FIN_Q) {
                s0 += (double)src[(size_t)b * stride];
                s1 += (double)src[(size_t)(b + RD_FIN_Q) * stride];
            }
            if (b < nblk) s0 += (double)src[(size_t)b * stride];
        }
    } else {
        const long c = ((long)blockIdx.x - g_blocks) * RD_FIN_E + el;
        if (c < Mg)
            for (int b = q; b < nblk; b += RD_FIN_Q) s0 += part_cs[(size_t)b * MgPad + c];
    }
    red[q][el] = s0 + s1;
    __syncthreads();
    if (q == 0) {
        double s = red[0][el];
#pragma unroll
        for (int i = 1; i < RD_FIN_Q; ++i) s += red[i][el];
        if (!is_cs) {
            if (e < total) {
                const int m = (int)(e / Ng), n = (int)(e - (long)m * Ng);
                float* d = G + (size_t)m * ldg + n;
                *d = accumulate ? (*d + (float)s) : (float)s;
            }
        } else {
            const long c = ((long)blockIdx.x - g_blocks) * RD_FIN_E + el;
            if (c < Mg) colsum[c] = accumulate ? (colsum[c] + (float)s) : (float)s;
        }
    }
}

const GpeRdSwitches& gpe_rd_switches()
{
    static const GpeRdSwitches sw = {gpe_dbg_env("GPE_RD_DEEP", -1), gpe_dbg_env("GPE_RD_NOPC", 0)};
    return sw;
}

extern "C" long gpe_redgemm_ws(int Mg, int Ng) { return gpe_rd_ws_floats(Mg, Ng); }

static int rd_launch_thin(const RdParams& p, const GpeRdPlan& plan, hipStream_t s)
{
    const size_t lds = (size_t)4 * p.MgPad * 5 * sizeof(float);
    if (plan.ql <= 1) { GPE_ENSURE_MAX_LDS((gpe_redgemm_thin_kernel<1>)); hipLaunchKernelGGL(gpe_redgemm_thin_kernel<1>, dim3(plan.gx), dim3(256), lds, s, p); }
    else if (plan.ql == 2) { GPE_ENSURE_MAX_LDS((gpe_redgemm_thin_kernel<2>)); hipLaunchKernelGGL(gpe_redgemm_thin_kernel<2>, dim3(plan.gx), dim3(256), lds, s, p); }
    else { GPE_ENSURE_MAX_LDS((gpe_redgemm_thin_kernel<4>)); hipLaunchKernelGGL(gpe_redgemm_thin_kernel<4>, dim3(plan.gx), dim3(256), lds, s, p); }
    GPE_CHECK_LAUNCH();
    return GPE_OK;
}

static int rd_launch_deep(const RdParams& p, const GpeRdPlan& plan, hipStream_t s)
{
    const size_t lds = (size_t)4 * RD_RT * RDD_LD * sizeof(float);
    const dim3 grid(plan.gx, plan.gy, plan.gz);
    if (plan.vvec) hipLaunchKernelGGL(gpe_redgemm_deep_kernel<true>, grid, dim3(256), lds, s, p);
    else hipLaunchKernelGGL(gpe_redgemm_deep_kernel<false>, grid, dim3(256), lds, s, p);
    GPE_CHECK_LAUNCH();
    return GPE_OK;
}

template <int MT, int NT, int VMODE, bool F16 = false, bool LAZY = false>
static int rd_b3_launch(const RdParams& p, int gx, hipStream_t s)
{
    const size_t lds = (size_t)2 * (RdB3Layout<MT>::BYTES + RdB3Layout<NT>::BYTES);
    GPE_ENSURE_MAX_LDS((gpe_redgemm_b3_kernel<MT, NT, VMODE, F16, LAZY>));
    hipLaunchKernelGGL((gpe_redgemm_b3_kernel<MT, NT, VMODE, F16, LAZY>), dim3(gx), dim3(512), lds, s, p);
    GPE_CHECK_LAUNCH();
    return GPE_OK;
}

template <int MT, int NT, int VMODE>
static int rd_pc_launch(const RdParams& p, int gx, hipStream_t s)
{
    constexpr int UC = 16 * MT, VC = 16 * NT;
    constexpr int LDU = (UC % 32 == 16) ? UC : UC + 16;
    constexpr int LDV = (VC % 32 == 16) ? VC : VC + 16;
    const size_t lds = (size_t)2 * RD_RT * (LDU + LDV) * sizeof(float);
    GPE_ENSURE_MAX_LDS((gpe_redgemm_pc_kernel<MT, NT, VMODE>));
    hipLaunchKernelGGL((gpe_redgemm_pc_kernel<MT, NT, VMODE>), dim3(gx), dim3(512), lds, s, p);
    GPE_CHECK_LAUNCH();
    return GPE_OK;
}

template <int MH, int NH, int VMODE>
static int rd_big_launch(const RdParams& p, dim3 grid, hipStream_t s)
{
    const size_t lds = (size_t)2 * RD_RT * ((32 * MH + 16) + (32 * NH + 16)) * sizeof(float);
    GPE_ENSURE_MAX_LDS((gpe_redgemm_kernel<MH, NH, VMODE>));
    hipLaunchKernelGGL((gpe_redgemm_kernel<MH, NH, VMODE>), grid, dim3(256), lds, s, p);
    GPE_CHECK_LAUNCH();
    return GPE_OK;
}

static int rd_launch_b3_lazy(const RdParams& p, const GpeRdPlan& plan, hipStream_t s)
{
    return (plan.MT == 13) ? rd_b3_launch<13, 13, V_DENSE, true, true>(p, plan.gx, s) : rd_b3_launch<10, 13, V_DENSE, true, true>(p, plan.gx, s);
}

static int rd_launch_b3_f16(const RdParams& p, const GpeRdPlan& plan, hipStream_t s)
{
    if (plan.MT == 13 && plan.vmode == V_DENSE) return rd_b3_launch<13, 13, V_DENSE, true>(p, plan.gx, s);
    if (plan.MT == 13) return rd_b3_launch<13, 13, V_GATHER, true>(p, plan.gx, s);
    if (plan.vmode == V_DENSE) return rd_b3_launch<10, 13, V_DENSE, true>(p, plan.gx, s);
    return rd_b3_launch<10, 13, V_GATHER, true>(p, plan.gx, s);
}
static int rd_launch_b3_bf16(const RdParams& p, const GpeRdPlan& plan, hipStream_t s)
{
    if (plan.MT == 13 && plan.vmode == V_DENSE) return rd_b3_launch<13, 13, V_DENSE>(p, plan.gx, s);
    if (plan.MT == 13) return rd_b3_launch<13, 13, V_GATHER>(p, plan.gx, s);
    if (plan.vmode == V_DENSE) return rd_b3_launch<10, 13, V_DENSE>(p, plan.gx, s);
    return rd_b3_launch<10, 13, V_GATHER>(p, plan.gx, s);
}
static int rd_launch_pc(const RdParams& p, const GpeRdPlan& plan, hipStream_t s)
{
    if (plan.MT == 13 && plan.vmode == V_DENSE) return rd_pc_launch<13, 13, V_DENSE>(p, plan.gx, s);
    if (plan.MT == 13) return rd_pc_launch<13, 13, V_GATHER>(p, plan.gx, s);
    if (plan.vmode == V_DENSE) return rd_pc_launch<10, 13, V_DENSE>(p, plan.gx, s);
    return rd_pc_launch<10, 13, V_GATHER>(p, plan.gx, s);
}

template <int VMODE>
static int rd_big_menu(const RdParams& p, const GpeRdPlan& plan, hipStream_t s)
{
    const dim3 grid(plan.gx, plan.gy);
#define RD_CASE(M_, N_) if (plan.MH == M_ && plan.NH == N_) return rd_big_launch<M_, N_, VMODE>(p, grid, s)
    RD_CASE(2, 1); RD_CASE(2, 5); RD_CASE(2, 7); RD_CASE(2, 8);
    RD_CASE(5, 1); RD_CASE(5, 5); RD_CASE(5, 7); RD_CASE(5, 8);
    RD_CASE(7, 1); RD_CASE(7, 5); RD_CASE(7, 7); RD_CASE(7, 8);
#undef RD_CASE
    return GPE_EINVAL;
}
static int rd_launch_big(const RdParams& p, const GpeRdPlan& plan, hipStream_t s)
{
    return (plan.vmode == V_DENSE) ? rd_big_menu<V_DENSE>(p, plan, s) : rd_big_menu<V_GATHER>(p, plan, s);
}

static int rd_finish(const RdParams& p, const GpeRdPlan& plan, float* G, int ldG, float* colsum, int accumulate, hipStream_t s)
{
    const long blocks = gpe_cdiv((long)p.Mg * p.Ng, RD_FIN_E) + (colsum ? gpe_cdiv(p.Mg, RD_FIN_E) : 0);
    hipLaunchKernelGGL(gpe_redgemm_finish, dim3(blocks), dim3(RD_FIN_E * RD_FIN_Q), 0, s, p.part, p.part_cs, plan.nblk, p.Mg, p.Ng,
                       plan.MgPad, plan.NgPad, G, ldG, colsum, accumulate);
    GPE_CHECK_LAUNCH();
    return GPE_OK;
}

static GpeRdPlan rd_plan(const RdParams& p, int vmode, bool want_colsum)
{
    return gpe_redgemm_plan(p, vmode, want_colsum, gpe_math_redgemm(), gpe_debug_get(), gpe_rd_switches(), gpe_num_cus());
}

static int rd_run(RdParams& p, int vmode, float* G, int ldG, float* colsum, float* part, int accumulate, hipStream_t s)
{
    const GpeRdPlan plan = rd_plan(p, vmode, colsum != nullptr);
    if (plan.path == GPE_RD_NOTHING) return plan.rc;
    p.vec = plan.vec; p.MgPad = plan.MgPad; p.NgPad = plan.NgPad; p.num_tiles = plan.num_tiles;
    p.umagic = plan.umagic; p.vmagic = plan.vmagic; p.pin_tpc = plan.pin_tpc;
    p.part = part;
    p.part_cs = plan.cs ? reinterpret_cast<double*>(part + plan.cs_off) : nullptr;
    int rc = GPE_EINVAL;
    switch (plan.path) {
    case GPE_RD_THIN: rc = rd_launch_thin(p, plan, s); break;
    case GPE_RD_X6_TN: rc = gpe_gemm_x6_launch_redgemm(p, plan, s); break;
    case GPE_RD_DEEP: rc = rd_launch_deep(p, plan, s); break;
    case GPE_RD_B3_LAZY: rc = rd_launch_b3_lazy(p, plan, s); break;
    case GPE_RD_B3_F16: rc = rd_launch_b3_f16(p, plan, s); break;
    case GPE_RD_B3_BF16: rc = rd_launch_b3_bf16(p, plan, s); break;
    case GPE_RD_PC: rc = rd_launch_pc(p, plan, s); break;
    case GPE_RD_BIG: rc = rd_launch_big(p, plan, s); break;
    default: break;
    }
    if (rc != GPE_OK) return rc;
    return rd_finish(p, plan, G, ldG, colsum, accumulate, s);
}

static bool rd_call_dense(RdParams& p, const float* u, long u_so, long u_si, int u_inner, const float* v, long v_so, long v_si, int v_inner,
                          long rows, int Mg, int Ng)
{
    if (!u || !v || rows < 0 || Mg <= 0 || Ng <= 0 || Ng > 256) return false;
    p.rows = rows; p.Mg = Mg; p.Ng = Ng;
    p.u = GpeRows{u, u_so, u_si, u_inner};
    p.v = GpeRows{v, v_so, v_si, v_inner};
    return true;
}
static bool rd_call_edge(RdParams& p, const float* u, int ldu, int v_mode, const float* v, int ldv, const float* pq, int ldpq, bool has_jg,
                         int B, int N, int k, int Mg, int Ng, bool lazy, bool has_amax_u, bool has_amax_v)
{
    if (!u || B <= 0 || N <= 0 || k <= 0 || Mg <= 0 || Ng <= 0 || Ng > 256 || ldu < Mg) return false;
    if (v_mode == 0 && (!pq || !has_jg || (Ng & 3) || (ldpq & 3))) return false;
    if ((long)B * N * k >= (1L << 31)) return false;
    if (v_mode == 1 && (!v || ldv < Ng)) return false;
    if (lazy && (k != 16 || v_mode != 1 || !has_amax_u || !has_amax_v)) return false;
    p.rows = (long)B * N * k; p.Mg = Mg; p.Ng = Ng;
    p.u = GpeRows{u, ldu, 0, 0};
    p.v = GpeRows{v, ldv, 0, 0};
    p.pq = pq; p.ldpq = ldpq; p.H = Ng; p.k = k; p.rcp_k = 1.0 / k; p.kmagic = (unsigned)(((1ull << 32) + k - 1) / k);
    p.pin_clouds = B;
    return true;
}

extern "C" int gpe_redgemm(const float* u, long u_so, long u_si, int u_inner, const float* v, long v_so,
                           long v_si, int v_inner, const float* v_shift, long rows, int Mg, int Ng, float* G,
                           int ldg, float* colsum, float* part, int accumulate, void* stream)
{
    RdParams p = {};
    if (!G || !part || ldg < Ng || !rd_call_dense(p, u, u_so, u_si, u_inner, v, v_so, v_si, v_inner, rows, Mg, Ng)) return GPE_EINVAL;
    p.v_shift = v_shift;
    return rd_run(p, V_DENSE, G, ldg, colsum, part, accumulate, (hipStream_t)stream);
}

extern "C" int gpe_edge_redgemm(const float* u, int ldu, int v_mode, const float* v, int ldv, const float* pq,
                                int ldpq, const int32_t* jg, const float* v_shift, int B, int N, int k, int Mg,
                                int Ng, float* G, int ldG, float* colsum, float* part, const uint32_t* amax_u,
                                const uint32_t* amax_v, void* ws, long ws_bytes, const float* lz_g, int lz_ldg,
                                const uint8_t* lz_amx, const uint8_t* lz_amn, int lz_ldagg, const float* lz_coef, void* stream)
{
    RdParams p = {};
    if (!G || !part || ldG < Ng || !rd_call_edge(p, u, ldu, v_mode, v, ldv, pq, ldpq, jg != nullptr, B, N, k, Mg, Ng, lz_g != nullptr,
                                                amax_u != nullptr, amax_v != nullptr))
        return GPE_EINVAL;
    p.jg = jg; p.v_shift = v_shift;
    if (lz_g) {
// ... 49 lines not shown
```

garment-pattern-estimation_amd/ops.py:

```python
import collections
import contextlib
import math
import os
import warnings
import weakref

import numpy as np
import torch

from . import _lib as L
from . import streams
from ._opbase import (F32, F64, _WS, _dev_check, _rows2d, _rows3d, _stitch_ldw, _ticket, _word, _workspace,
                      edge_workspace, f16x3_words, round_up)


def pack_fold(W, bias, stats, ews, ews_n, clear_word):
    N, K = W.shape
    wp = torch.empty(L.query('gpe_packed_size', N, K), device=W.device, dtype=F32)
    bf = torch.empty(N, device=W.device, dtype=F32)
    L.call('gpe_pack_fold', W, W.stride(0), N, K, stats[2], stats[3], bias, wp, bf, ews, ews_n if ews is not None else 0, clear_word,
           _ticket(W.device) if ews is not None else None)
    return wp, bf


SIDE_GRADS = not (os.environ.get('GPE_DEBUG') == '1' and os.environ.get('GPE_SIDE_GRADS') == '0')
SIDE_MIN_EDGES = 1 << 17
SIDE_PQ = not (os.environ.get('GPE_DEBUG') == '1' and os.environ.get('GPE_SIDE_PQ') == '0')
_LAST_EDGES = [0]


def _side_ok(edges):
    return bool(SIDE_GRADS and edges >= SIDE_MIN_EDGES and not torch.cuda.is_current_stream_capturing())


def side_grads(params, tensors):
    if params and _side_ok(_LAST_EDGES[0]) and all(_SINK.get(p.data_ptr()) is not None and _SINK[p.data_ptr()][0]() is not None for p in params):
        return streams.lane(params[0].device.index).fork(tensors, leaf=True)
    return contextlib.nullcontext(False)


WEIGHTS_EPOCH = 0
_PACKS = {}

K_PLAIN, K_TRANS, K_GATES, K_PQ, K_PQT, K_VADD, K_BPQ, K_GRUB = 0, 1, 2, 3, 4, 5, 6, 7
K_GATES_H3, K_AMAX, K_TRANS_H3 = 8, 9, 10
PLANE_KINDS = (K_GATES_H3, K_TRANS_H3)
_JOB = np.dtype([('w', '<u8'), ('w2', '<u8'), ('out', '<u8'), ('total', '<i8'), ('first_block', '<i8'),
                 ('ldw', '<i4'), ('N', '<i4'), ('K', '<i4'), ('kind', '<i4'), ('Npad', '<i4'), ('aux', '<i4')])
assert _JOB.itemsize == 64
PackSpec = collections.namedtuple('PackSpec', 'p p2 kind N K aux out_numel')


def _pack_geometry(sp):
    if sp.kind in (K_VADD, K_BPQ, K_GRUB):
        return 0, sp.out_numel
    if sp.kind in (K_GATES, K_GATES_H3):
        npad = 16 * (sp.N // sp.aux) * ((sp.aux + 15) // 16)
    else:
        npad = round_up(sp.N, 16)
    if sp.kind == K_GATES:
        return npad, npad * round_up(sp.K, 16)
    if sp.kind in PLANE_KINDS:
        return npad, L.query('gpe_packed_planes_size', npad, sp.K)
    return npad, L.query('gpe_packed_size', sp.N, sp.K)


def _job_table(rows, dev):
    tab = np.zeros(len(rows), dtype=_JOB)
    blk = 0
    for i, (w, w2, out, total, ldw, N, K, kind, npad, aux) in enumerate(rows):
        tab[i] = (w, w2, out, total, blk, ldw, N, K, kind, npad, aux)
        blk += L.query('gpe_pack_job_blocks', kind, total, npad, K)
    return torch.from_numpy(tab.view(np.uint8).copy()).to(dev), blk




def bump_weights_epoch():
    global WEIGHTS_EPOCH
    WEIGHTS_EPOCH += 1


class PackPlan:

    def __init__(self):
        self.specs = []
        self.outs = []
        self.table = None
        self.blocks = 0
        self.vers = None
        self.epoch = -1
        self.home = None
        self.keys = []
        self.frozen = False
        self.h3_current = False
# ... 193 lines not shown
    L.call('gpe_w1_split', W1, W1.stride(0), b1, H, C, wpq, C, bpq)
    return pack_weight(wpq), pack_weight(wpq, transpose=True), bpq


def fold_bias(w, bias, t):
    out = torch.empty(w.shape[0], device=w.device, dtype=F32)
    L.call('gpe_fold_bias', w, w.stride(0), w.shape[0], w.shape[1], bias, t, out)
    return out


def linear_raw(a_desc, wp, bias, M, N, K, y_desc, act=0, addend_desc=None):
    ad = addend_desc if addend_desc is not None else (None, 0, 0, 0)
    L.call('gpe_linear', a_desc[0], a_desc[1], a_desc[2], a_desc[3], wp, bias,
           ad[0], ad[1], ad[2], ad[3], y_desc[0], y_desc[1], y_desc[2], y_desc[3], M, N, K, act)


def redgemm_raw(u_desc, v_desc, rows, Mg, Ng, want_colsum=True, accumulate_into=None, v_shift=None, out=None):
    dev = u_desc[0].device
    if accumulate_into is not None:
        G, cs = accumulate_into
    elif out is not None:
        G, cs = out
    else:
        G = torch.empty(Mg, Ng, device=dev, dtype=F32)
        cs = torch.empty(Mg, device=dev, dtype=F32) if want_colsum else None
    acc = int(accumulate_into is not None)
    for n0 in range(0, Ng, 256):
        nb = min(256, Ng - n0)
        ws = torch.empty(L.query('gpe_redgemm_ws', Mg, nb), device=dev, dtype=F32)
        L.call('gpe_redgemm', u_desc[0], u_desc[1], u_desc[2], u_desc[3],
               v_desc[0][..., n0:], v_desc[1], v_desc[2], v_desc[3], None if v_shift is None else v_shift[n0:],
               rows, Mg, nb, G[:, n0:], G.stride(0), cs if n0 == 0 else None, ws, acc)
    return G, cs


def knn(x, B, N, k, want_global=False, order=None, want_order=False):
    _dev_check(x)
    idx = torch.empty(B, N, k, device=x.device, dtype=torch.int32)
    jg = torch.empty(B, N, k, device=x.device, dtype=torch.int32) if want_global else None
    oo = torch.empty(B, N, device=x.device, dtype=torch.int32) if want_order else None
    if order is not None:
        assert order.dtype == torch.int32 and order.shape == (B, N) and order.is_contiguous() and order.device == x.device
    nws = L.query('gpe_knn_ws_bytes', B, N, x.shape[1], k)
    L.call('gpe_knn', x, B, N, x.shape[1], x.stride(0), k, idx, jg, order, oo, _workspace(nws, x.device), nws)
    out = (idx, jg) if want_global else (idx,)
    if want_order:
        out = out + (oo,)
    return out if len(out) > 1 else out[0]


def knn_reverse(idx):
    B, N, k = idx.shape
    off = torch.empty(B, N + 1, device=idx.device, dtype=torch.int32)
    edge = torch.empty(B, N * k, device=idx.device, dtype=torch.int32)
    L.call('gpe_knn_reverse', idx, B, N, k, off, edge)
    return off, edge


def bn_finalize(part, nblk, C, count, gamma, beta, eps, momentum, rm, rv, nbt):
    stats = torch.empty(4, C, device=gamma.device, dtype=F32)
    L.call('gpe_bn_finalize', part, nblk, C, float(count), gamma, beta, float(eps), float(momentum), rm, rv, nbt,
           stats)
    return stats


def bn_from_running(rm, rv, gamma, beta, eps):
    C = gamma.shape[0]
    stats = torch.empty(4, C, device=gamma.device, dtype=F32)
    L.call('gpe_bn_from_running', rm, rv, C, gamma, beta, float(eps), stats)
    return stats


def bn_bwd_coef(part, nblk, stats, C, count, gamma=None, beta=None, training=True):
    dev = stats.device
    coef = torch.empty(4, C, device=dev, dtype=F32)
    dg = _gbuf(gamma) if gamma is not None else torch.empty(C, device=dev, dtype=F32)
    db = _gbuf(beta) if beta is not None else torch.empty(C, device=dev, dtype=F32)
    L.call('gpe_bn_bwd_coef', part, nblk, stats, C, float(count), coef, dg, db)
    if not training:
        coef[1:3].zero_()
    return coef, dg, db


def bn_stats(blk, eps, training=False, momentum=None, part=None, nblk=0, count=0):
    if training:
        return bn_finalize(part, nblk, blk.W.shape[0], count, blk.gamma, blk.beta, eps, momentum, blk.running_mean, blk.running_var,
                           blk.num_batches_tracked)
    return bn_from_running(blk.running_mean, blk.running_var, blk.gamma, blk.beta, eps)


MLP_PARAMS, MLP_BUFFERS = ('W', 'b', 'gamma', 'beta'), ('running_mean', 'running_var', 'num_batches_tracked')
MLPBlock = collections.namedtuple('MLPBlock', MLP_PARAMS + MLP_BUFFERS, defaults=(None,) * len(MLP_BUFFERS))


def mlp_tensors(mlp):
    blocks = [mlp[i] for i in range(len(mlp))]
    flat = [t for lin, _, bn in blocks for t in (lin.weight, lin.bias, bn.weight, bn.bias)]
    flat += [t for _, _, bn in blocks for t in (bn.running_mean, bn.running_var, bn.num_batches_tracked)]
    return blocks[0][2].eps, blocks[0][2].momentum, len(blocks), tuple(flat)


def mlp_blocks(tensors, nb):
    P, Q = len(MLP_PARAMS), len(MLP_BUFFERS)
    return [MLPBlock(*tensors[P * l: P * l + P], *tensors[P * nb + Q * l: P * nb + Q * l + Q]) for l in range(nb)]


def mlp_grads(lead, nb, filed=None, gx=None):
    out = [gx] + [None] * (lead - 1 + (len(MLP_PARAMS) + len(MLP_BUFFERS)) * nb)
    for (l, field), g in (filed or {}).items():
        out[lead + len(MLP_PARAMS) * l + MLP_PARAMS.index(field)] = g
    return tuple(out)


def save_groups(ctx, **groups):
    ctx.saved_groups = [(name, len(g) if isinstance(g, (list, tuple)) else None) for name, g in groups.items()]
    ctx.save_for_backward(*[t for g in groups.values() for t in (g if isinstance(g, (list, tuple)) else (g,))])


def saved_groups(ctx):
    sv, at, out = ctx.saved_tensors, 0, {}
    for name, n in ctx.saved_groups:
        out[name] = sv[at] if n is None else list(sv[at: at + n])
        at += 1 if n is None else n
    return out


EdgeSrc = collections.namedtuple('EdgeSrc', 'pq ldpq jg t ld')
NO_LAZY = (None, 0, None, None, 0, None)


def edge_gathered(PQ, jg):
    return EdgeSrc(PQ, PQ.stride(0), jg, None, 0)


def edge_rows(t):
    return EdgeSrc(None, 0, None, t, t.stride(0))


def edge_mlp_fwd(*, src, dims, Cin, Cout, wp, bias, out, ldo, stats_part, agg, ldagg, amax_a, amax_out, ws, out_half):
    mx, mn, amx, amn = agg or (None, None, None, None)
    L.call('gpe_edge_mlp_fwd', int(src.pq is None), *src, *dims, Cin, Cout, wp, bias, out, ldo, stats_part, int(agg is not None),
           mx, mn, amx, amn, ldagg, amax_a, amax_out, *ws, out_half)


def edge_redgemm(*, u, ldu, v, v_shift, dims, Mg, Ng, G, ldG, colsum, part, amax_u, amax_v, ws, lazy=NO_LAZY):
    L.call('gpe_edge_redgemm', u, ldu, int(v.pq is None), v.t, v.ld, v.pq, v.ldpq, v.jg, v_shift, *dims, Mg, Ng, G, ldG, colsum, part,
           amax_u, amax_v, *ws, *lazy)


def edge_mlp_bwd(*, a, lda, act, dims, Cin, Cout, wp, coef, out, ldo, dP, lddp, amax_a, amax_out, ws, lazy=NO_LAZY):
    pq, ldpq, jg = (None, 0, None) if act is None else act[:3]
    L.call('gpe_edge_mlp_bwd', a, lda, int(act is not None), pq, ldpq, jg, *dims, Cin, Cout, wp, coef, out, ldo, dP, lddp,
           amax_a, amax_out, *ws, *lazy)


def _block_bwd(filed, blocks, l, dz, src, st_prev, dims, count, training, amax, ws, part, lazy=NO_LAZY, first=None):
    W, b, gp, bp = blocks[l].W, blocks[l].b, blocks[l - 1].gamma, blocks[l - 1].beta
    Cl, Cp = W.shape[0], blocks[l - 1].W.shape[0]
    G = torch.empty(Cl, Cp, device=W.device, dtype=F32)
    db = _gbuf(b)
    if part is None:
        redgemm_raw((dz, dz.stride(0), 0, 0), (src.t, src.ld, 0, 0), count, Cl, Cp, v_shift=st_prev[0], out=(G, db))
    else:
        edge_redgemm(u=dz, ldu=dz.stride(0), v=src, v_shift=st_prev[0], dims=dims, Mg=Cl, Ng=Cp, G=G, ldG=Cp, colsum=db, part=part,
                     amax_u=amax[0], amax_v=amax[1], ws=ws, lazy=lazy)
    sums = torch.empty(1, 2, Cp, device=W.device, dtype=torch.float64)
    dW = _gbuf(W)
    L.call('gpe_bn_bwd_from_G', G, Cp, db, W, W.stride(0), Cl, Cp, st_prev, sums, dW, Cp)
    coef_p, dgp, dbp = bn_bwd_coef(sums, 1, st_prev, Cp, count, gp, bp, training)
    filed[l, 'W'], filed[l, 'b'] = _gret(W, dW), _gret(b, db)
    filed[l - 1, 'gamma'], filed[l - 1, 'beta'] = _gret(gp, dgp), _gret(bp, dbp)
    (out, ldo), (dP, lddp) = ((src.t, src.ld), (None, 0)) if first is None else ((first[0], Cp), (first[1], first[1].stride(0)))
    edge_mlp_bwd(a=dz, lda=dz.stride(0), act=None if first is None else src, dims=dims, Cin=Cl, Cout=Cp,
                 wp=pack_weight(W, transpose=True), coef=coef_p, out=out, ldo=ldo, dP=dP, lddp=lddp, amax_a=amax[0], amax_out=amax[2],
                 ws=ws, lazy=lazy)
    return out


class LinearFn(torch.autograd.Function):

    @staticmethod
    def forward(ctx, x, weight, bias):
        _dev_check(x)
        K = x.shape[-1]
        M = x.numel() // K
        N = weight.shape[0]
        y = torch.empty(M, N, device=x.device, dtype=F32)
        linear_raw(_rows3d(x) if x.dim() == 3 else _rows2d(x), pack_weight(weight), bias, M, N, K, _rows2d(y))
        ctx.save_for_backward(x, weight, bias)
        return y

    @staticmethod
    def backward(ctx, gy):
        x, weight, bias = ctx.saved_tensors
        gy = gy.contiguous()
        K = x.shape[-1]
        M = x.numel() // K
        N = weight.shape[0]
        xd = _rows3d(x) if x.dim() == 3 else _rows2d(x)
        gx = gw = gb = None
        if ctx.needs_input_grad[0]:
            gx = torch.empty(*x.shape, device=x.device, dtype=F32)
            linear_raw(_rows2d(gy), pack_weight(weight, transpose=True), None, M, K, N, (gx, K, 0, 0))
        if ctx.needs_input_grad[1] or bias is not None:
            with side_grads([weight, bias] if bias is not None else [], [gy, x]):
                gw = _gbuf(weight)
                gb = _gbuf(bias) if bias is not None else torch.empty(N, device=x.device, dtype=F32)
                redgemm_raw(_rows2d(gy), xd, M, N, K, out=(gw, gb))
                gw = _gret(weight, gw)
                gb = _gret(bias, gb) if bias is not None else None
        return gx, gw, gb


def linear(x, weight, bias=None):
    return LinearFn.apply(x, weight, bias)


POOL_MODES = {'mean': 0, 'max': 1, 'add': 2}


class SegmentMeanFn(torch.autograd.Function):

    @staticmethod
    def forward(ctx, x, B, N):
        _dev_check(x)
        C = x.shape[1]
        y = torch.empty(B, C, device=x.device, dtype=F32)
        L.call('gpe_segment_mean_fwd', x, x.stride(0), B, N, C, y, C)
        ctx.dims = (B, N, C)
        return y

    @staticmethod
    def backward(ctx, gy):
        B, N, C = ctx.dims
        gy = gy.contiguous()
        gx = torch.empty(B * N, C, device=gy.device, dtype=F32)
        L.call('gpe_segment_mean_bwd', gy, C, B, N, C, gx, C, 0)
        return gx, None, None


class SegmentPoolFn(torch.autograd.Function):

    @staticmethod
    def forward(ctx, x, B, N, mode):
        _dev_check(x)
        C = x.shape[1]
        y = torch.empty(B, C, device=x.device, dtype=F32)
        arg = torch.empty(B, C, device=x.device, dtype=torch.int32) if mode == 1 else None
        L.call('gpe_segment_pool_fwd', x, x.stride(0), B, N, C, mode, y, C, arg)
        ctx.dims = (B, N, C, mode)
        ctx.arg = arg
        return y
# ... 182 lines not shown
            agg = None
            if last and aggr == 'max':
                mx = torch.empty(BN, ldo, device=dev, dtype=F32)
                mn = torch.empty(BN, ldo, device=dev, dtype=F32)
                amx = torch.empty(BN, ldo, device=dev, dtype=torch.uint8)
                amn = torch.empty(BN, ldo, device=dev, dtype=torch.uint8)
                agg = (mx, mn, amx, amn)
            w_out = _word(words, l)
            wp, bf = pack_fold(blocks[l].W, blocks[l].b, stats[l - 1], ews[0] if words is not None else None, ews[1], w_out)
            wr = 2 if words is not None else 0
            src = edge_gathered(PQ, jg) if l == 1 else edge_rows(acts[l - 1])

            def launch(a, out_half):
                edge_mlp_fwd(src=src, dims=(B, N, k), Cin=Cin, Cout=Cout, wp=wp, bias=bf, out=a, ldo=ldo, stats_part=part, agg=agg,
                             ldagg=ldo, amax_a=_word(words, l - 1), amax_out=w_out, ws=ews, out_half=out_half)

            launch(a, int(half) | wr)
            if half and guard is not None and not guard.watch(w_out):
                a = torch.empty(E, ldo, device=dev, dtype=F32)
                launch(a, 0)
            acts.append(a)
            stats.append(bn_stats(blocks[l], eps, training, momentum, part, nblk, E))
        Fo = widths[-1]
        ldF = round_up(Fo, 4)
        out = torch.empty(BN, ldF, device=dev, dtype=F32)[:, :Fo]
        if aggr == 'max':
            L.call('gpe_edge_finish', mx, mn, ldF, stats[-1], BN, Fo, out, ldF)
        else:
            abar = torch.empty(BN, ldF, device=dev, dtype=F32)
            L.call('gpe_edge_sum_k', acts[-1], ldF, BN, k, Fo, abar, ldF)
            L.call('gpe_scale', abar, 1.0 / k, abar, abar.numel())
            a_s, t_s = (1.0, 1.0) if aggr == 'mean' else (float(k), float(k))
            L.call('gpe_bn_apply_scaled', abar, ldF, stats[-1], BN, Fo, a_s, t_s, out, ldF)
        ctx.dims = (B, N, k, C, nb, aggr, training)
        ctx.widths = widths
        ctx.done = False
        ctx.words = words
        ctx.rev_job = None
        if fork and training:
            if order is None:
                del lane.jobs[:]
            ctx.rev_job = {'fn': knn_reverse, 'src': idx, 'out': None, 'event': None}
            lane.jobs.append(ctx.rev_job)
        save_groups(ctx, x=x, idx=idx, jg=jg, PQ=PQ, params=tensors[:len(MLP_PARAMS) * nb], acts=acts[1:], stats=stats,
                    tail=[mx, mn, amx, amn] if aggr == 'max' else [abar])
        ctx.mark_non_differentiable(idx, order_out)
        return out, idx, order_out

    @staticmethod
    def backward(ctx, g_out, _g_idx, _g_order=None):
        if ctx.done:
            raise RuntimeError('EdgeConvFn.backward ran twice on the same graph: the stored activations are overwritten '
                               'in place by the first pass (retain_graph is not supported)')
        B, N, k, C, nb, aggr, training = ctx.dims
        if g_out is None:
            return mlp_grads(EdgeConvFn.LEAD, nb)
        ctx.done = True
        widths = ctx.widths
        sv = saved_groups(ctx)
        x, idx, jg, PQ, stats, tail = sv['x'], sv['idx'], sv['jg'], sv['PQ'], sv['stats'], sv['tail']
        blocks = mlp_blocks(sv['params'], nb)
        acts = [None] + sv['acts']
        dev = x.device
        BN, E = B * N, B * N * k
        H0, Fo = widths[0], widths[-1]
        ldF = round_up(Fo, 4)
        if g_out.stride(1) != 1:
            g_out = g_out.contiguous()
        ldg = g_out.stride(0)
        filed = {}
        words = ctx.words
        ews = edge_workspace(B, N, k, max(ldF, 2 * H0), dev)
        rev, rev_event = None, None
        job = getattr(ctx, 'rev_job', None)
        lane = streams.lane(dev.index)
        if job is not None and job['out'] is not None:
            rev, rev_event = job['out'], job['event']
        elif SIDE_PQ and _side_ok(E):
            if job is not None and job in lane.jobs:
                lane.jobs.remove(job)
            with lane.fork([idx]):
                rev = knn_reverse(idx)

        psb = L.query('gpe_point_sums_blocks')
        part = torch.empty(psb, 2, Fo, device=dev, dtype=torch.float64)
        g_last, be_last = blocks[-1].gamma, blocks[-1].beta
        a_last = acts[-1]
        lz = NO_LAZY
        if aggr == 'max':
            mx, mn, amx, amn = tail
            lazy = a_last.dtype == torch.float16 and L.query('gpe_edge_lazy_dz3_ok', B, N, k, Fo, widths[-2]) == 1
            if a_last.dtype == torch.float16 and not lazy:
                a_last = a_last.float()
            L.call('gpe_edge_bwd_point_sums', g_out, ldg, mx, mn, ldF, stats[-1], BN, Fo, part,
                   _word(words, 2 * nb) if lazy else None)
            coef, dg, dbe = bn_bwd_coef(part, psb, stats[-1], Fo, E, g_last, be_last, training)
            if lazy:
                L.call('gpe_edge_dz3_bound', _word(words, 2 * nb), coef, Fo, _word(words, nb - 1), _word(words, 2 * nb - 1))
                lz = (g_out, ldg, amx, amn, ldF, coef)
            else:
                L.call('gpe_edge_dz3', a_last, ldF, g_out, ldg, amx, amn, ldF, coef, B, N, k, Fo, _word(words, 2 * nb - 1))
        else:
            abar, = tail
            gs = g_out
            if aggr == 'add':
                gs = torch.empty(BN, Fo, device=dev, dtype=F32)
                L.call('gpe_scale', g_out.contiguous(), float(k), gs, gs.numel())
            L.call('gpe_edge_bwd_point_sums', gs, gs.stride(0), abar, abar, ldF, stats[-1], BN, Fo, part, None)
            coef, dg, dbe = bn_bwd_coef(part, psb, stats[-1], Fo, E, g_last, be_last, training)
            L.call('gpe_edge_dz3_all', a_last, ldF, g_out, ldg, 1.0 / k if aggr == 'mean' else 1.0, coef, B, N, k, Fo,
                   _word(words, 2 * nb - 1))
        filed[nb - 1, 'gamma'], filed[nb - 1, 'beta'] = _gret(g_last, dg), _gret(be_last, dbe)

        ws = torch.empty(max(L.query('gpe_redgemm_ws', widths[l], widths[l - 1]) for l in range(1, nb)), device=dev,
                         dtype=F32)
        dPQ = torch.empty(BN, 2 * H0, device=dev, dtype=F32)
        dz = a_last
        for l in range(nb - 1, 1, -1):
            dz = _block_bwd(filed, blocks, l, dz, edge_rows(acts[l - 1]), stats[l - 1], (B, N, k), E, training,
                            (_word(words, nb + l), _word(words, l - 1), _word(words, nb + l - 1)), ews, ws,
                            lazy=lz if l == nb - 1 else NO_LAZY)
        dst = dz if dz.stride(0) == H0 else torch.empty(E, H0, device=dev, dtype=F32)
        dz = _block_bwd(filed, blocks, 1, dz, edge_gathered(PQ, jg), stats[0], (B, N, k), E, training,
                        (_word(words, nb + 1), _word(words, 0), None), ews, ws, first=(dst, dPQ))

        if rev is not None:
            rev_off, rev_edge = rev
            lane.wait(made=rev, event=rev_event)
        else:
            rev_off, rev_edge = knn_reverse(idx)
        L.call('gpe_edge_pull_dq', dz, dz.stride(0), rev_off, rev_edge, B, N, k, H0, dPQ[:, H0:], 2 * H0)
        dWpq, dbpq = redgemm_raw(_rows2d(dPQ), _rows2d(x), BN, 2 * H0, C, want_colsum=True)
        W1, b1 = blocks[0].W, blocks[0].b
        dW1 = _gbuf(W1)
        L.call('gpe_w1_grad_from_pq', dWpq, C, H0, C, dW1, 2 * C)
        db1 = _gbuf(b1)
        db1.copy_(dbpq[:H0])
        filed[0, 'W'], filed[0, 'b'] = _gret(W1, dW1), _gret(b1, db1)
        gx = None
        if ctx.needs_input_grad[0]:
            _, wpq_t, _ = edge_first_operands(W1, b1)
            gx = torch.empty(BN, C, device=dev, dtype=F32)
            linear_raw(_rows2d(dPQ), wpq_t, None, BN, C, 2 * H0, _rows2d(gx))
        return mlp_grads(EdgeConvFn.LEAD, nb, filed, gx)


class EdgeInputsFn(torch.autograd.Function):

    @staticmethod
    def forward(ctx, x, idx, jg, B, N, k):
        _dev_check(x)
        C = x.shape[1]
        ld = round_up(2 * C, 4)
        out = torch.empty(B * N * k, ld, device=x.device, dtype=F32)
        L.call('gpe_edge_inputs_fwd', x, x.stride(0), C, jg, B * N, k, out, ld)
        ctx.save_for_backward(idx)
        ctx.dims = (B, N, k, C)
        return out[:, :2 * C]

    @staticmethod
    def backward(ctx, g):
        idx, = ctx.saved_tensors
        B, N, k, C = ctx.dims
        if g.stride(1) != 1:
            g = g.contiguous()
        rev_off, rev_edge = knn_reverse(idx)
        gx = torch.empty(B * N, C, device=g.device, dtype=F32)
        L.call('gpe_edge_inputs_bwd', g, g.stride(0), C, rev_off, rev_edge, B, N, k, gx, C)
        return gx, None, None, None, None, None


def edge_conv_general(x, B, N, k, training, eps, momentum, nb, aggr, tensors):
    idx, jg = knn(x, B, N, k, want_global=True)
    msg_in = EdgeInputsFn.apply(x, idx, jg, B, N, k)
    msg = DenseMLPFn.apply(msg_in, training, eps, momentum, nb, *tensors)
    if aggr == 'max':
        out = SegmentPoolFn.apply(msg, B * N, k, 1)
    elif aggr == 'add':
        out = SegmentPoolFn.apply(msg, B * N, k, 2)
    else:
        out = SegmentMeanFn.apply(msg, B * N, k)
    return out, idx


EDGE_PREDICT_ROUTES = ('auto', 'fused', 'layers')
EDGE_PREDICT_MAX_K, EDGE_PREDICT_MAX_WIDTH, EDGE_PREDICT_MAX_HIDDEN, EDGE_PREDICT_H3_MAX_WIDTH = 64, 256, 3, 224
_AGGR_CODE = {'max': 0, 'mean': 1, 'add': 2}


def _edge_widths_on_menu(shapes, k):
    nb = len(shapes)
    if nb < 2 or nb - 2 > EDGE_PREDICT_MAX_HIDDEN or not 1 <= k <= EDGE_PREDICT_MAX_K:
# ... 348 lines not shown
    noise = torch.empty(T, Bn, H).bernoulli_(1 - p).div_(1 - p)
    return noise.transpose(0, 1).contiguous().to(device, non_blocking=True)


def rnn_stack(x, h0, c0, T, n_layers, kind, params, want_state=False, dropout=0.0, training=False, h0_bounded=False):
    h0_ok = True
    if not h0_bounded and L.get_math() == 'f16x3' and h0 is not None:
        h0_ok = bool(h0.abs().max().item() < 16.0)
    if not (dropout > 0 and training and n_layers > 1):
        out = RNNStackFn.apply(x, h0, c0, T, n_layers, kind, want_state, h0_ok, *params)
        return out if kind == 'lstm' else (out[0], out[1], None)
    lstm = kind == 'lstm'
    layers = rnn_layers(params, n_layers)
    inp, hs, cs = x, [], []
    for l in range(n_layers):
        out = RNNStackFn.apply(inp, h0[l:l + 1], c0[l:l + 1] if lstm else None, T, 1, kind, want_state, h0_ok, *layers[l])
        top = out[0]
        if want_state:
            hs.append(out[1])
            if lstm:
                cs.append(out[2])
        if l < n_layers - 1:
            inp = DropoutMulFn.apply(top, _dropout_mask(T, top.shape[0], top.shape[2], float(dropout), top.device))
    hN = torch.cat(hs, 0) if want_state else None
    cN = torch.cat(cs, 0) if (want_state and lstm) else None
    return top, hN, cN


class DenseMLPFn(torch.autograd.Function):
    LEAD = 5

    @staticmethod
    def forward(ctx, x, training, eps, momentum, n_blocks, *tensors):
        _dev_check(x)
        dev = x.device
        M = x.shape[0]
        nblk = L.query('gpe_stats_blocks')
        acts, stats = [], []
        a_in, Cin = x, x.shape[1]
        scale = tvec = None
        ews = edge_workspace(1, M, 1, 4, dev)
        words = f16x3_words(2 * n_blocks, M, dev)
        for l, blk in enumerate(mlp_blocks(tensors, n_blocks)):
            W, b = blk.W, blk.b
            Cout = W.shape[0]
            ldo = round_up(Cout, 4)
            a = torch.empty(M, ldo, device=dev, dtype=F32)
            part = torch.empty(nblk, 2, Cout, device=dev, dtype=torch.float64) if training else None
            edge_mlp_fwd(src=edge_rows(a_in), dims=(1, M, 1), Cin=Cin, Cout=Cout, wp=pack_weight(W, col_scale=scale),
                         bias=b if tvec is None else fold_bias(W, b, tvec), out=a, ldo=ldo, stats_part=part, agg=None, ldagg=0,
                         amax_a=_word(words, l - 1) if l > 0 else None, amax_out=_word(words, l) if l < n_blocks - 1 else None,
                         ws=ews, out_half=0)
            st = bn_stats(blk, eps, training, momentum, part, nblk, M)
            acts.append(a)
            stats.append(st)
            scale, tvec = st[2], st[3]
            a_in, Cin = a, Cout
        y = torch.empty(M, Cin, device=dev, dtype=F32)
        L.call('gpe_bn_apply', a_in, a_in.stride(0), stats[-1], M, Cin, y, Cin)
        ctx.n_blocks = n_blocks
        ctx.training = training
        ctx.done = False
        ctx.words = words
        save_groups(ctx, x=x, params=tensors[:len(MLP_PARAMS) * n_blocks], acts=acts, stats=stats)
        return y

    @staticmethod
    def backward(ctx, gy):
        if ctx.done:
            raise RuntimeError('DenseMLPFn.backward ran twice on the same graph: the stored activations are overwritten '
                               'in place by the first pass (retain_graph is not supported)')
        ctx.done = True
        n, training = ctx.n_blocks, ctx.training
        sv = saved_groups(ctx)
        x, acts, stats = sv['x'], sv['acts'], sv['stats']
        blocks = mlp_blocks(sv['params'], n)
        dev = x.device
        M = x.shape[0]
        gy = gy.contiguous()
        filed = {}
        a, st = acts[-1], stats[-1]
        C = blocks[-1].W.shape[0]
        g_l, be_l = blocks[-1].gamma, blocks[-1].beta
        psb = L.query('gpe_point_sums_blocks')
        part = torch.empty(psb, 2, C, device=dev, dtype=torch.float64)
        L.call('gpe_edge_bwd_point_sums', gy, C, a, a, a.stride(0), st, M, C, part, None)
        coef, dgam, dbet = bn_bwd_coef(part, psb, st, C, M, g_l, be_l, training)
        words = ctx.words
        ews = edge_workspace(1, M, 1, 4, dev)
        L.call('gpe_edge_dz3_all', a, a.stride(0), gy, C, 1.0, coef, 1, M, 1, C, _word(words, 2 * n - 1))
        filed[n - 1, 'gamma'], filed[n - 1, 'beta'] = _gret(g_l, dgam), _gret(be_l, dbet)
        dz = a
        for l in range(n - 1, 0, -1):
            Cl, Cp = blocks[l].W.shape[0], blocks[l - 1].W.shape[0]
            ws = None if Cp > 256 else torch.empty(L.query('gpe_redgemm_ws', Cl, Cp), device=dev, dtype=F32)
            dz = _block_bwd(filed, blocks, l, dz, edge_rows(acts[l - 1]), stats[l - 1], (1, M, 1), M, training,
                            (_word(words, n + l), _word(words, l - 1), _word(words, n + l - 1)), ews, ws)
        W0, b0 = blocks[0].W, blocks[0].b
        H0, K0 = W0.shape[0], x.shape[1]
        dW, db = _gbuf(W0), _gbuf(b0)
        redgemm_raw((dz, dz.stride(0), 0, 0), _rows2d(x), M, H0, K0, out=(dW, db))
        filed[0, 'W'], filed[0, 'b'] = _gret(W0, dW), _gret(b0, db)
        gx = None
        if ctx.needs_input_grad[0]:
            gx = torch.empty(M, K0, device=dev, dtype=F32)
            linear_raw((dz, dz.stride(0), 0, 0), pack_weight(W0, transpose=True), None, M, K0, H0, _rows2d(gx))
        return mlp_grads(DenseMLPFn.LEAD, n, filed, gx)


def dense_mlp(x, mlp, training):
    x = x if x.stride(1) == 1 else x.contiguous()
    eps, momentum, n, tensors = mlp_tensors(mlp)
    return DenseMLPFn.apply(x, training, eps, momentum, n, *tensors)


class SparsemaxFn(torch.autograd.Function):

    @staticmethod
    def forward(ctx, z):
        _dev_check(z)
        z = z.contiguous()
        M, W = z.shape
        out = torch.empty_like(z)
        L.call('gpe_sparsemax_fwd', z, W, M, W, out, W)
        ctx.save_for_backward(out)
        return out

    @staticmethod
    def backward(ctx, g):
        out, = ctx.saved_tensors
        g = g.contiguous()
        M, W = out.shape
        gz = torch.empty_like(out)
        L.call('gpe_sparsemax_bwd', out, W, g, W, M, W, gz, W)
        return gz


class AttentionPoolFn(torch.autograd.Function):

    @staticmethod
    def forward(ctx, w, feat, B, N, mode=0):
        _dev_check(w)
        dev = w.device
        P, C = w.shape[1], feat.shape[1]
        pooled = torch.empty(B, P, C, device=dev, dtype=F32)
        nws = L.query('gpe_attn_pool_ws', B, N, P, C)
        part = torch.empty(nws, device=dev, dtype=F32)
        arg = torch.empty(B, P, C, device=dev, dtype=torch.int32) if mode == 1 else None
        part_arg = torch.empty(nws, device=dev, dtype=torch.int32) if mode == 1 else None
        L.call('gpe_attn_pool_fwd', w, w.stride(0), feat, feat.stride(0), B, N, P, C, mode, pooled, arg, part, part_arg)
        ctx.dims = (B, N, P, C, mode)
        ctx.arg = arg
        ctx.save_for_backward(w, feat)
        return pooled.view(B * P, C)

    @staticmethod
    def backward(ctx, g):
        w, feat = ctx.saved_tensors
        B, N, P, C, mode = ctx.dims
        dev = w.device
        g = g.contiguous()
        gw = torch.empty(B * N, P, device=dev, dtype=F32)
        gf = torch.empty(B * N, C, device=dev, dtype=F32)
        L.call('gpe_attn_pool_bwd', w, w.stride(0), feat, feat.stride(0), g, ctx.arg, B, N, P, C, mode, gw, P, gf, C)
        return gw, gf, None, None, None


def fps_start(B, N, device):
    start = (torch.rand(B) * float(N)).long().clamp_(max=N - 1)
    return start.to(torch.int32).to(device, non_blocking=True)
# ... 64 lines not shown
```

Baseline: 3808 garments/s.

## Fuse BN-backward coefficient chains, kNN prologue, and vectorise amax and redgemm finish

Adds a fused point-sums+BN-coefficient kernel that uses ticketed chained workgroups to reduce the partial sums and produce coef/dgamma/dbeta in one launch. It also folds the BN coefficient step into gpe_bn_bwd_from_G and adds a single kNN prologue kernel that computes norms, per-cloud max, fp16 split planes and identity order together. Smaller changes vectorise the f16x3 amax scan with uint4 loads and add a 4-wide redgemm finish kernel. The goal is fewer eager launches and less memory traffic per step, at the cost of cross-workgroup ticket synchronisation and several new code paths.

```diff
diff --git a/garment-pattern-estimation_amd/_lib.py b/garment-pattern-estimation_amd/_lib.py
--- a/garment-pattern-estimation_amd/_lib.py
+++ b/garment-pattern-estimation_amd/_lib.py
@@ -17,6 +17,8 @@
 PLACE_HEADERS = (PLACE_HEADER_PATH,)
 FRAMEWORK_HEADER_PATH = os.path.join(os.path.dirname(_HERE), 'include', 'gpe_hip_framework.h')
 FRAMEWORK_HEADERS = (FRAMEWORK_HEADER_PATH,)
+CHAIN_HEADER_PATH = os.path.join(os.path.dirname(_HERE), 'include', 'gpe_hip_chain.h')
+CHAIN_HEADERS = (CHAIN_HEADER_PATH,)
 
 _CT = {'p': ctypes.c_void_p, 'i': ctypes.c_int, 'l': ctypes.c_long, 'f': ctypes.c_float, 'd': ctypes.c_double}
 
@@ -61,7 +63,7 @@
                 'libgpe_hip.so not built: run `python -c "import __graft_entry__ as g; g.build()"` '
                 '(hipcc --offload-arch=gfx950).  There is no CPU fallback for the product path.')
         l = ctypes.CDLL(LIB_PATH)
-        for header in HEADERS + FEATURE_HEADERS + EVAL_HEADERS + PLACE_HEADERS + FRAMEWORK_HEADERS:
+        for header in HEADERS + FEATURE_HEADERS + EVAL_HEADERS + PLACE_HEADERS + FRAMEWORK_HEADERS + CHAIN_HEADERS:
             for name, (res, args) in parse_header(header).items():
                 fn = getattr(l, name)
                 fn.restype = _CT[res]
diff --git a/garment-pattern-estimation_amd/_opbase.py b/garment-pattern-estimation_amd/_opbase.py
--- a/garment-pattern-estimation_amd/_opbase.py
+++ b/garment-pattern-estimation_amd/_opbase.py
@@ -76,6 +76,17 @@
     return t
 
 
+_CHAIN_TICKETS = {}
+
+
+def _chain_tickets(n, device):
+    key = streams.stream_key(device)
+    t = _CHAIN_TICKETS.get(key)
+    if t is None or t.numel() < n:
+        t = _CHAIN_TICKETS[key] = torch.zeros(max(int(n), 64), device=torch.device('cuda', key[0]), dtype=torch.int32)
+    return t
+
+
 def _stitch_ldw(H):
     nb = (H + 15) // 16
     nb = 4 if nb <= 4 else 8 if nb <= 8 else 13 if nb <= 13 else 16
diff --git a/garment-pattern-estimation_amd/build.py b/garment-pattern-estimation_amd/build.py
--- a/garment-pattern-estimation_amd/build.py
+++ b/garment-pattern-estimation_amd/build.py
@@ -30,7 +30,7 @@
     inc = os.path.join(os.path.dirname(HERE), 'include')
     deps = [os.path.join(CSRC, src), os.path.abspath(__file__)]
     deps += [os.path.join(inc, h) for h in ('gpe_hip.h', 'gpe_hip_ext.h', 'gpe_hip_fit.h', 'gpe_hip_eval.h', 'gpe_hip_place.h',
-                                              'gpe_hip_framework.h')]
+                                              'gpe_hip_framework.h', 'gpe_hip_chain.h')]
     deps += [os.path.join(CSRC, h) for h in os.listdir(CSRC) if h.endswith('.h')]
     return any(os.path.getmtime(d) > t for d in deps)
 
diff --git a/garment-pattern-estimation_amd/csrc/gpe_common.h b/garment-pattern-estimation_amd/csrc/gpe_common.h
--- a/garment-pattern-estimation_amd/csrc/gpe_common.h
+++ b/garment-pattern-estimation_amd/csrc/gpe_common.h
@@ -8,6 +8,7 @@
 #include "../../include/gpe_hip_eval.h"
 #include "../../include/gpe_hip_place.h"
 #include "../../include/gpe_hip_framework.h"
+#include "../../include/gpe_hip_chain.h"
 
 #define GPE_OK 0
 #define GPE_EINVAL (-22)
diff --git a/garment-pattern-estimation_amd/csrc/gpe_device.h b/garment-pattern-estimation_amd/csrc/gpe_device.h
--- a/garment-pattern-estimation_amd/csrc/gpe_device.h
+++ b/garment-pattern-estimation_amd/csrc/gpe_device.h
@@ -3,6 +3,7 @@
 #include <math.h>
 
 typedef _Float16 gpe_f16x2 __attribute__((ext_vector_type(2)));
+typedef _Float16 gpe_f16x4 __attribute__((ext_vector_type(4)));
 typedef _Float16 gpe_f16x8 __attribute__((ext_vector_type(8)));
 typedef __bf16 gpe_bf16x2 __attribute__((ext_vector_type(2)));
 typedef __bf16 gpe_bf16x8 __attribute__((ext_vector_type(8)));
diff --git a/garment-pattern-estimation_amd/csrc/gpe_edgegemm_h3.hip b/garment-pattern-estimation_amd/csrc/gpe_edgegemm_h3.hip
--- a/garment-pattern-estimation_amd/csrc/gpe_edgegemm_h3.hip
+++ b/garment-pattern-estimation_amd/csrc/gpe_edgegemm_h3.hip
@@ -65,7 +65,21 @@
 {
     __shared__ unsigned red[16];
     unsigned m = 0u;
-    for (long t = threadIdx.x; t < n; t += 1024) {
+    const long n4 = gpe_aligned16(w) ? (n >> 2) : 0;
+    const uint4* w4 = reinterpret_cast<const uint4*>(w);
+    for (long t0 = threadIdx.x; t0 < n4; t0 += 8 * 1024) {
+        uint4 q[8];
+#pragma unroll
+        for (int u = 0; u < 8; ++u) q[u] = w4[(t0 + u * 1024 < n4) ? t0 + u * 1024 : t0];
+#pragma unroll
+        for (int u = 0; u < 8; ++u) {
+            const unsigned a0 = q[u].x & 0x7fffffffu, a1 = q[u].y & 0x7fffffffu, a2 = q[u].z & 0x7fffffffu, a3 = q[u].w & 0x7fffffffu;
+            const unsigned b0 = a0 > a1 ? a0 : a1, b1 = a2 > a3 ? a2 : a3;
+            const unsigned b = b0 > b1 ? b0 : b1;
+            m = m > b ? m : b;
+        }
+    }
+    for (long t = (n4 << 2) + threadIdx.x; t < n; t += 1024) {
         const unsigned a = __float_as_uint(w[t]) & 0x7fffffffu;
         m = m > a ? m : a;
     }
diff --git a/garment-pattern-estimation_amd/csrc/gpe_knn.hip b/garment-pattern-estimation_amd/csrc/gpe_knn.hip
--- a/garment-pattern-estimation_amd/csrc/gpe_knn.hip
+++ b/garment-pattern-estimation_amd/csrc/gpe_knn.hip
@@ -690,6 +690,110 @@
                 row[CP + c] = l;
             }
         }
+    }
+}
+
+template <bool VEC4, bool PLANES>
+__global__ __launch_bounds__(256) void gpe_knn_prologue_kernel(const float* __restrict__ x, long rows, int N, int C, int ldx, int CP,
+                                                               float* __restrict__ norms, int* __restrict__ cmax,
+                                                               _Float16* __restrict__ pl, float* __restrict__ isc,
+                                                               const int* __restrict__ order, int* __restrict__ order_out)
+{
+    constexpr int R = KNN_NORM_ROWS;
+    __shared__ float nrmS[4 * R];
+    __shared__ int clS[4 * R];
+    const int lane = threadIdx.x & 63, wave = threadIdx.x >> 6;
+    const long r0 = ((long)blockIdx.x * 4 + wave) * R;
+    const long last = rows - 1;
+    int my_src, my_cl;
+    {
+        const long rr = r0 + (lane < R ? lane : 0);
+        const long r = rr < last ? rr : last;
+        const int b = (int)(r / N);
+        int o = (int)(r - (long)b * N);
+        if (order_out && lane < R && rr <= last) order_out[rr] = o;
+        if (order) { o = order[r]; o = o < 0 ? 0 : (o >= N ? N - 1 : o); }
+        my_src = b * N + o;
+        my_cl = (lane < R && rr <= last) ? b : -1;
+    }
+    float my_norm = 0.f;
+    const int c4 = 4 * lane;
+    float4 v[R];
+    float s[R], m[R];
+#pragma unroll
+    for (int u = 0; u < R; ++u) { s[u] = 0.f; m[u] = 0.f; }
+    for (int c0 = 0; c0 < C; c0 += 256) {
+        const int c = c0 + c4;
+#pragma unroll
+        for (int u = 0; u < R; ++u) {
+            const float* row = x + (long)__builtin_amdgcn_readlane(my_src, u) * ldx;
+            if (VEC4) {
+                v[u] = *reinterpret_cast<const float4*>(row + (c < C ? c : 0));
+            } else {
+                v[u].x = row[c < C ? c : 0];
+                v[u].y = row[c + 1 < C ? c + 1 : 0];
+                v[u].z = row[c + 2 < C ? c + 2 : 0];
+                v[u].w = row[c + 3 < C ? c + 3 : 0];
+            }
+        }
+#pragma unroll
+        for (int u = 0; u < R; ++u) {
+            v[u].x = (c < C) ? v[u].x : 0.f;
+            v[u].y = (c + 1 < C) ? v[u].y : 0.f;
+            v[u].z = (c + 2 < C) ? v[u].z : 0.f;
+            v[u].w = (c + 3 < C) ? v[u].w : 0.f;
+            s[u] = __builtin_fmaf(v[u].w, v[u].w, __builtin_fmaf(v[u].z, v[u].z, __builtin_fmaf(v[u].y, v[u].y, __builtin_fmaf(v[u].x, v[u].x, s[u]))));
+            if (PLANES) m[u] = fmaxf(fmaxf(fmaxf(m[u], fabsf(v[u].x)), fabsf(v[u].y)), fmaxf(fabsf(v[u].z), fabsf(v[u].w)));
+        }
+        if (PLANES) break;
+    }
+#pragma unroll
+    for (int u = 0; u < R; ++u) {
+        const bool live = r0 + u <= last;
+        float t = s[u];
+#pragma unroll
+        for (int o = 32; o > 0; o >>= 1) t += __int_as_float(__builtin_amdgcn_ds_bpermute((lane ^ o) << 2, __float_as_int(t)));
+        my_norm = (lane == u) ? t : my_norm;
+        if (lane == 0 && live) norms[__builtin_amdgcn_readlane(my_src, u)] = t;
+        if (PLANES) {
+            float mm = m[u];
+#pragma unroll
+            for (int o = 32; o > 0; o >>= 1) mm = fmaxf(mm, __int_as_float(__builtin_amdgcn_ds_bpermute((lane ^ o) << 2, __float_as_int(mm))));
+            float sc, inv;
+            gpe_h3_scale_of(__float_as_uint(mm), sc, inv);
+            if (lane == 0 && live) isc[r0 + u] = inv;
+            if (live && c4 < CP) {
+                const float xs[4] = {v[u].x * sc, v[u].y * sc, v[u].z * sc, v[u].w * sc};
+                gpe_f16x4 h, l;
+#pragma unroll
+                for (int e = 0; e < 4; ++e) {
+                    h[e] = (_Float16)xs[e];
+                    l[e] = (_Float16)(xs[e] - (float)h[e]);
+                }
+                _Float16* prow = pl + (r0 + u) * 2 * (long)CP;
+                *reinterpret_cast<gpe_f16x4*>(prow + c4) = h;
+                *reinterpret_cast<gpe_f16x4*>(prow + CP + c4) = l;
+            }
+        }
+    }
+    if (lane < R) { nrmS[wave * R + lane] = fmaxf(0.f, my_norm); clS[wave * R + lane] = my_cl; }
+    __syncthreads();
+    if (wave != 0) return;
+    const int cl = clS[lane];
+    float mx = cl >= 0 ? nrmS[lane] : 0.f;
+    const int cl0 = __builtin_amdgcn_readfirstlane(cl);
+    int lead = -1;
+    if (__all(cl < 0 || cl == cl0)) {
+#pragma unroll
+        for (int o = 32; o > 0; o >>= 1) mx = fmaxf(mx, __int_as_float(__builtin_amdgcn_ds_bpermute((lane ^ o) << 2, __float_as_int(mx))));
+        if (lane == 0) lead = cl0;
+    } else if (cl >= 0 && (lane == 0 || clS[lane - 1] != cl)) {
+        for (int j = lane + 1; j < 4 * R && clS[j] == cl; ++j) mx = fmaxf(mx, nrmS[j]);
+        lead = cl;
+    }
+    if (lead >= 0) {
+        const int bits = __float_as_int(mx);
+        if (bits > __hip_atomic_load(cmax + lead, __ATOMIC_RELAXED, __HIP_MEMORY_SCOPE_AGENT)) atomicMax(cmax + lead, bits);
     }
 }
 
@@ -1146,9 +1250,22 @@
 int gpe_knn_launch_prologue(const GpeKnnCall& c, const GpeKnnPlan& p)
 {
     const long nq = (long)c.B * c.N;
-    if (p.identity) {
+    const bool fused = p.fused && p.norms, own_identity = p.identity && !(fused && c.order_out != p.order);
+    if (own_identity) {
         hipLaunchKernelGGL(gpe_knn_identity_order_kernel, dim3((unsigned)gpe_cdiv(nq, 256)), dim3(256), 0, c.stream, c.order_out, nq, c.N);
         GPE_CHECK_LAUNCH();
+    }
+    if (fused) {
+        static_assert(4 * KNN_NORM_ROWS == 64, "the fused prologue's workgroup reduces its 4 x KNN_NORM_ROWS rows in one wave");
+        if (hipMemsetAsync(p.cmax, 0, gpe_knn_up256((size_t)c.B * sizeof(int)), c.stream) != hipSuccess) return GPE_ELAUNCH;
+        auto go = [&](auto kernel) {
+            hipLaunchKernelGGL(kernel, dim3((unsigned)gpe_cdiv(nq, 4 * KNN_NORM_ROWS)), dim3(256), 0, c.stream, c.x, nq, c.N, c.C, c.ldx,
+                               p.CP, p.norms, p.cmax, p.planes, p.iscale, p.order, (p.identity && !own_identity) ? c.order_out : nullptr);
+        };
+        if (p.planes) { if (p.pvec4) go(gpe_knn_prologue_kernel<true, true>); else go(gpe_knn_prologue_kernel<false, true>); }
+        else { if (p.pvec4) go(gpe_knn_prologue_kernel<true, false>); else go(gpe_knn_prologue_kernel<false, false>); }
+        GPE_CHECK_LAUNCH();
+        return GPE_OK;
     }
     if (p.norms) {
         hipLaunchKernelGGL(gpe_knn_norms_kernel, dim3((unsigned)gpe_cdiv(nq, 4 * KNN_NORM_ROWS)), dim3(256), 0, c.stream, c.x, nq, c.N, c.C,
diff --git a/garment-pattern-estimation_amd/csrc/gpe_knn_plan.h b/garment-pattern-estimation_amd/csrc/gpe_knn_plan.h
--- a/garment-pattern-estimation_amd/csrc/gpe_knn_plan.h
+++ b/garment-pattern-estimation_amd/csrc/gpe_knn_plan.h
@@ -26,6 +26,7 @@
     int NOORDER;
     int FT;
     int RR2;
+    int PROLOGUE;
 };
 const GpeKnnSwitches& gpe_knn_switches();
 
@@ -79,6 +80,7 @@
 struct GpeKnnPlan {
     GpeKnnPath path; int rc;
     bool identity;
+    bool fused, pvec4;
     int pin, tiles, nsplit, vec;
     long nblocks;
     int probe; bool smallc;
@@ -173,6 +175,8 @@
     p.part = (unsigned long long*)scratch;
     p.norms = (float*)(scratch + w.norms);
     p.cmax = (int*)(scratch + w.cmax);
+    p.fused = sw.PROLOGUE != 0;
+    p.pvec4 = c.ldx % 4 == 0 && (uintptr_t)c.x % 16 == 0 && ((c.C + 3) & ~3) <= c.ldx;
     p.CP = (c.C + 31) & ~31;
     p.NB = p.CP >> 5;
     p.ce = (6.f * c.C + (h3 ? 32.f : 16.f)) * 5.9604645e-8f;
diff --git a/garment-pattern-estimation_amd/csrc/gpe_knn_search.hip b/garment-pattern-estimation_amd/csrc/gpe_knn_search.hip
--- a/garment-pattern-estimation_amd/csrc/gpe_knn_search.hip
+++ b/garment-pattern-estimation_amd/csrc/gpe_knn_search.hip
@@ -5,7 +5,7 @@
     static const GpeKnnSwitches sw = {gpe_dbg_env("GPE_KNN_PROBE", 0),  gpe_dbg_env("GPE_KNN_PIN", -1),  gpe_dbg_env("GPE_KNN_VEC", 0),
                                       gpe_dbg_env("GPE_KNN_SPLIT", 0),  gpe_dbg_env("GPE_KNN_EXACT", 0), gpe_dbg_env("GPE_KNN_F32FILTER", 0),
                                       gpe_dbg_env("GPE_KNN_SORTED", 1), gpe_dbg_env("GPE_KNN_NOORDER", 0), gpe_dbg_env("GPE_KNN_FT", 1),
-                                      gpe_dbg_env("GPE_KNN_RR2", 1)};
+                                      gpe_dbg_env("GPE_KNN_RR2", 1),    gpe_dbg_env("GPE_KNN_PROLOGUE", 1)};
     return sw;
 }
 
diff --git a/garment-pattern-estimation_amd/csrc/gpe_pointwise.hip b/garment-pattern-estimation_amd/csrc/gpe_pointwise.hip
--- a/garment-pattern-estimation_amd/csrc/gpe_pointwise.hip
+++ b/garment-pattern-estimation_amd/csrc/gpe_pointwise.hip
@@ -621,11 +621,20 @@
 }
 
 #define PS_BLOCKS 512
-__global__ __launch_bounds__(256) void gpe_point_sums_kernel(const float* __restrict__ g, int ldg,
-                                                             const float* __restrict__ mx,
-                                                             const float* __restrict__ mn, int ldagg,
-                                                             const float* __restrict__ stats, long rows, int C,
-                                                             double* __restrict__ part, unsigned* __restrict__ amax_sg)
+__device__ __forceinline__ void ps_store_sc1(double* p, double v)
+{
+    __hip_atomic_store(reinterpret_cast<unsigned long long*>(p), (unsigned long long)__double_as_longlong(v), __ATOMIC_RELAXED,
+                       __HIP_MEMORY_SCOPE_AGENT);
+}
+__device__ __forceinline__ double ps_load_sc1(const double* p)
+{
+    return __longlong_as_double((long long)__hip_atomic_load(reinterpret_cast<const unsigned long long*>(p), __ATOMIC_RELAXED,
+                                                             __HIP_MEMORY_SCOPE_AGENT));
+}
+template <bool SC1>
+__device__ __forceinline__ void point_sums_body(const float* __restrict__ g, int ldg, const float* __restrict__ mx,
+                                                const float* __restrict__ mn, int ldagg, const float* __restrict__ stats, long rows,
+                                                int C, double* __restrict__ part, unsigned* __restrict__ amax_sg)
 {
     const int c = blockIdx.y * 256 + threadIdx.x;
     double s1 = 0, s2 = 0;
@@ -653,8 +662,13 @@
             s2 += (double)gv * (double)((sel - mean) * rstd);
             gm = fmaxf(gm, fabsf(gv));
         }
-        part[(size_t)blockIdx.x * 2 * C + c] = s1;
-        part[(size_t)blockIdx.x * 2 * C + C + c] = s2;
+        if (SC1) {
+            ps_store_sc1(part + (size_t)blockIdx.x * 2 * C + c, s1);
+            ps_store_sc1(part + (size_t)blockIdx.x * 2 * C + C + c, s2);
+        } else {
+            part[(size_t)blockIdx.x * 2 * C + c] = s1;
+            part[(size_t)blockIdx.x * 2 * C + C + c] = s2;
+        }
         sabs = fabsf(s);
     }
     if (amax_sg) {
@@ -663,6 +677,14 @@
         for (int o = 32; o > 0; o >>= 1) m = fmaxf(m, __shfl_xor(m, o));
         if ((threadIdx.x & 63) == 0) atomicMax(amax_sg, __float_as_uint(m * 1.0000002f));
     }
+}
+__global__ __launch_bounds__(256) void gpe_point_sums_kernel(const float* __restrict__ g, int ldg,
+                                                             const float* __restrict__ mx,
+                                                             const float* __restrict__ mn, int ldagg,
+                                                             const float* __restrict__ stats, long rows, int C,
+                                                             double* __restrict__ part, unsigned* __restrict__ amax_sg)
+{
+    point_sums_body<false>(g, ldg, mx, mn, ldagg, stats, rows, C, part, amax_sg);
 }
 
 extern "C" int gpe_point_sums_blocks(void) { return PS_BLOCKS; }
@@ -720,6 +742,100 @@
     return GPE_OK;
 }
 
+#define PSC_CHAIN_BLOCKS (PS_BLOCKS / BNC_WAVES)
+static_assert(PS_BLOCKS % BNC_WAVES == 0, "every chain of the fused point sums has the same number of workgroups");
+__global__ __launch_bounds__(256) void gpe_point_sums_coef_kernel(const float* __restrict__ g, int ldg, const float* __restrict__ mx,
+                                                                  const float* __restrict__ mn, int ldagg,
+                                                                  const float* __restrict__ stats, long rows, int C, double count,
+                                                                  double* part, double* chain_ws, float* __restrict__ coef,
+                                                                  float* dgamma, float* dbeta, unsigned* amax_sg,
+                                                                  const unsigned* __restrict__ amax_a3, unsigned* amax_out,
+                                                                  unsigned* tickets)
+{
+    __shared__ int last_sh;
+    __shared__ float bred[4];
+    point_sums_body<true>(g, ldg, mx, mn, ldagg, stats, rows, C, part, amax_sg);
+    const int w = blockIdx.x % BNC_WAVES;
+    gpe_drain_stores();
+    __syncthreads();
+    if (threadIdx.x == 0) last_sh = gpe_flag_ticket(tickets + 1 + blockIdx.y * BNC_WAVES + w) == PSC_CHAIN_BLOCKS - 1;
+    __syncthreads();
+    if (!last_sh) return;
+    __builtin_amdgcn_fence(__ATOMIC_ACQUIRE, "agent");
+    const int c = blockIdx.y * 256 + threadIdx.x;
+    if (c < C) {
+        double v1[PSC_CHAIN_BLOCKS], v2[PSC_CHAIN_BLOCKS];
+#pragma unroll
+        for (int i = 0; i < PSC_CHAIN_BLOCKS; ++i) {
+            v1[i] = ps_load_sc1(part + (size_t)(w + i * BNC_WAVES) * 2 * C + c);
+            v2[i] = ps_load_sc1(part + (size_t)(w + i * BNC_WAVES) * 2 * C + C + c);
+        }
+        double s1 = 0, s2 = 0;
+#pragma unroll
+        for (int i = 0; i < PSC_CHAIN_BLOCKS; ++i) { s1 += v1[i]; s2 += v2[i]; }
+        ps_store_sc1(chain_ws + (size_t)w * 2 * C + c, s1);
+        ps_store_sc1(chain_ws + (size_t)w * 2 * C + C + c, s2);
+    }
+    gpe_drain_stores();
+    __syncthreads();
+    if (threadIdx.x == 0) last_sh = gpe_flag_ticket(tickets) == gridDim.y * BNC_WAVES - 1;
+    __syncthreads();
+    if (!last_sh) return;
+    __builtin_amdgcn_fence(__ATOMIC_ACQUIRE, "agent");
+    const float a3 = amax_out ? __uint_as_float(amax_a3[0]) * 1.001f : 0.f;
+    float tail = 0.f;
+    for (int cc = threadIdx.x; cc < C; cc += 256) {
+        double s1 = 0, s2 = 0;
+        for (int w_ = 0; w_ < BNC_WAVES; ++w_) {
+            s1 += ps_load_sc1(chain_ws + (size_t)w_ * 2 * C + cc);
+            s2 += ps_load_sc1(chain_ws + (size_t)w_ * 2 * C + C + cc);
+        }
+        const double mean = stats[cc], rstd = stats[C + cc], s = stats[2 * C + cc];
+        const double m1 = s1 / count, m2 = s2 / count;
+        const double k2 = s * rstd * m2;
+        const float f_c1 = (float)(s * m1), f_k2 = (float)k2, f_mean = (float)mean;
+        coef[cc] = (float)s;
+        coef[C + cc] = f_c1;
+        coef[2 * C + cc] = f_k2;
+        coef[3 * C + cc] = f_mean;
+        if (dgamma) dgamma[cc] = (float)s2;
+        if (dbeta) dbeta[cc] = (float)s1;
+        tail = fmaxf(tail, fabsf(f_c1) + (a3 + fabsf(f_mean)) * fabsf(f_k2));
+    }
+    if (amax_out) {
+#pragma unroll
+        for (int o = 32; o > 0; o >>= 1) tail = fmaxf(tail, __shfl_xor(tail, o));
+        if ((threadIdx.x & 63) == 0) bred[threadIdx.x >> 6] = tail;
+    }
+    __syncthreads();
+    if (threadIdx.x == 0) {
+        if (amax_out) {
+            tail = fmaxf(fmaxf(bred[0], bred[1]), fmaxf(bred[2], bred[3]));
+            const float sg = __uint_as_float(__hip_atomic_load(amax_sg, __ATOMIC_RELAXED, __HIP_MEMORY_SCOPE_AGENT));
+            const float b = (sg + tail) * 1.000001f;
+            amax_out[0] = __float_as_uint(b) & 0x7fffffffu;
+        }
+    }
+    for (int t = threadIdx.x; t < 1 + (int)gridDim.y * BNC_WAVES; t += 256)
+        __hip_atomic_store(tickets + t, 0u, __ATOMIC_RELAXED, __HIP_MEMORY_SCOPE_AGENT);
+}
+
+extern "C" int gpe_point_sums_coef_tickets(int C) { return C > 0 ? 1 + gpe_cdiv(C, 256) * BNC_WAVES : GPE_EINVAL; }
+
+extern "C" int gpe_edge_bwd_point_sums_coef(const float* g, int ldg, const float* mx, const float* mn, int ldagg, const float* stats,
+                                            long rows, int C, double count, double* part, double* chain_ws, float* coef,
+                                            float* dgamma, float* dbeta, uint32_t* amax_sg, const uint32_t* amax_a3,
+                                            uint32_t* amax_out, uint32_t* tickets, void* stream)
+{
+    if (!g || !mx || !mn || !stats || !part || !chain_ws || !coef || !tickets || rows <= 0 || C <= 0 || !(count > 0)) return GPE_EINVAL;
+    if ((amax_sg || amax_a3 || amax_out) && !(amax_sg && amax_a3 && amax_out)) return GPE_EINVAL;
+    if (amax_sg && hipMemsetAsync(amax_sg, 0, sizeof(uint32_t), (hipStream_t)stream) != hipSuccess) return GPE_ELAUNCH;
+    hipLaunchKernelGGL(gpe_point_sums_coef_kernel, dim3(PS_BLOCKS, gpe_cdiv(C, 256)), dim3(256), 0, (hipStream_t)stream, g, ldg, mx, mn,
+                       ldagg, stats, rows, C, count, part, chain_ws, coef, dgamma, dbeta, amax_sg, amax_a3, amax_out, tickets);
+    GPE_CHECK_LAUNCH();
+    return GPE_OK;
+}
+
 #define DZ3_RB 8
 __global__ __launch_bounds__(256) void gpe_dz3_kernel(float* __restrict__ a3, int lda3, const float* __restrict__ g,
                                                       int ldg, const uint8_t* __restrict__ amx,
@@ -824,9 +940,11 @@
 }
 
 #define BNG_FQ 16
-__global__ __launch_bounds__(64 * BNG_FQ) void gpe_bn_bwd_from_G_kernel(
+template <bool COEF>
+__device__ __forceinline__ void bn_bwd_from_G_body(
     const float* __restrict__ G, int ldG, const float* __restrict__ db, const float* __restrict__ w, int ldw, int Cn,
-    int C, const float* __restrict__ stats, double* __restrict__ sums, float* __restrict__ dw, int lddw)
+    int C, const float* __restrict__ stats, double* __restrict__ sums, float* __restrict__ dw, int lddw, double count,
+    float* __restrict__ coef, float* dgamma, float* dbeta)
 {
     __shared__ double red[BNG_FQ][2][64];
     const int lane = threadIdx.x & 63, fq = threadIdx.x >> 6;
@@ -862,8 +980,35 @@
     if (fq != 0 || c >= C) return;
     a = 0; b = 0;
     for (int q = 0; q < BNG_FQ; ++q) { a += red[q][0][lane]; b += red[q][1][lane]; }
-    sums[c] = a;
-    sums[C + c] = b * (double)stats[C + c];
+    b *= (double)stats[C + c];
+    if (sums) { sums[c] = a; sums[C + c] = b; }
+    if (COEF) {
+        double s1 = 0, s2 = 0;
+        s1 += a;
+        s2 += b;
+        const double mean = stats[c], rstd = stats[C + c], s = stats[2 * C + c];
+        const double m1 = s1 / count, m2 = s2 / count;
+        const double k2 = s * rstd * m2;
+        coef[c] = (float)s;
+        coef[C + c] = (float)(s * m1);
+        coef[2 * C + c] = (float)k2;
+        coef[3 * C + c] = (float)mean;
+        if (dgamma) dgamma[c] = (float)s2;
+        if (dbeta) dbeta[c] = (float)s1;
+    }
+}
+__global__ __launch_bounds__(64 * BNG_FQ) void gpe_bn_bwd_from_G_kernel(
+    const float* __restrict__ G, int ldG, const float* __restrict__ db, const float* __restrict__ w, int ldw, int Cn,
+    int C, const float* __restrict__ stats, double* __restrict__ sums, float* __restrict__ dw, int lddw)
+{
+    bn_bwd_from_G_body<false>(G, ldG, db, w, ldw, Cn, C, stats, sums, dw, lddw, 1.0, nullptr, nullptr, nullptr);
+}
+__global__ __launch_bounds__(64 * BNG_FQ) void gpe_bn_bwd_from_G_coef_kernel(
+    const float* __restrict__ G, int ldG, const float* __restrict__ db, const float* __restrict__ w, int ldw, int Cn,
+    int C, const float* __restrict__ stats, double* __restrict__ sums, float* __restrict__ dw, int lddw, double count,
+    float* __restrict__ coef, float* dgamma, float* dbeta)
+{
+    bn_bwd_from_G_body<true>(G, ldG, db, w, ldw, Cn, C, stats, sums, dw, lddw, count, coef, dgamma, dbeta);
 }
 
 extern "C" int gpe_bn_bwd_from_G(const float* G, int ldG, const float* db, const float* w_next, int ldw, int Cn,
@@ -872,6 +1017,18 @@
     if (!G || !db || !w_next || !stats || !sums || Cn <= 0 || C <= 0 || ldG < C || ldw < C) return GPE_EINVAL;
     hipLaunchKernelGGL(gpe_bn_bwd_from_G_kernel, dim3(gpe_cdiv(C, 64)), dim3(64 * BNG_FQ), 0, (hipStream_t)stream, G, ldG, db,
                        w_next, ldw, Cn, C, stats, sums, dw, lddw);
+    GPE_CHECK_LAUNCH();
+    return GPE_OK;
+}
+
+extern "C" int gpe_bn_bwd_from_G_coef(const float* G, int ldG, const float* db, const float* w_next, int ldw, int Cn, int C,
+                                      const float* stats, double count, double* sums, float* dw, int lddw, float* coef,
+                                      float* dgamma, float* dbeta, void* stream)
+{
+    if (!G || !db || !w_next || !stats || !coef || Cn <= 0 || C <= 0 || ldG < C || ldw < C || !(count > 0)) return GPE_EINVAL;
+    if (dw && lddw < C) return GPE_EINVAL;
+    hipLaunchKernelGGL(gpe_bn_bwd_from_G_coef_kernel, dim3(gpe_cdiv(C, 64)), dim3(64 * BNG_FQ), 0, (hipStream_t)stream, G, ldG, db,
+                       w_next, ldw, Cn, C, stats, sums, dw, lddw, count, coef, dgamma, dbeta);
     GPE_CHECK_LAUNCH();
     return GPE_OK;
 }
diff --git a/garment-pattern-estimation_amd/csrc/gpe_redgemm.hip b/garment-pattern-estimation_amd/csrc/gpe_redgemm.hip
--- a/garment-pattern-estimation_amd/csrc/gpe_redgemm.hip
+++ b/garment-pattern-estimation_amd/csrc/gpe_redgemm.hip
@@ -1130,6 +1130,79 @@
     }
 }
 
+__global__ __launch_bounds__(RD_FIN_E * RD_FIN_Q) void gpe_redgemm_finish4(
+    const float* __restrict__ part, const double* __restrict__ part_cs, int nblk, int Mg, int Ng, int MgPad, int NgPad,
+    float* G, int ldg, float* colsum, int accumulate)
+{
+    __shared__ double red[RD_FIN_Q][RD_FIN_E][4];
+    const int el = threadIdx.x & (RD_FIN_E - 1), q = threadIdx.x / RD_FIN_E;
+    const int ng4 = (Ng + 3) >> 2;
+    const long total = (long)Mg * ng4;
+    const long e = (long)blockIdx.x * RD_FIN_E + el;
+    const long g_blocks = (total + RD_FIN_E - 1) / RD_FIN_E;
+    const bool is_cs = (long)blockIdx.x >= g_blocks;
+    double s0[4] = {0, 0, 0, 0}, s1[4] = {0, 0, 0, 0};
+    if (!is_cs) {
+        if (e < total) {
+            const int m = (int)(e / ng4), n0 = 4 * (int)(e - (long)m * ng4);
+            const size_t stride = (size_t)MgPad * NgPad;
+            const float* src = part + (size_t)m * NgPad + n0;
+            int b = q;
+            for (; b + 7 * RD_FIN_Q < nblk; b += 8 * RD_FIN_Q) {
+                float4 v[8];
+#pragma unroll
+                for (int u = 0; u < 8; ++u) v[u] = *reinterpret_cast<const float4*>(src + (size_t)(b + u * RD_FIN_Q) * stride);
+#pragma unroll
+                for (int u = 0; u < 8; u += 2) {
+                    s0[0] += (double)v[u].x; s0[1] += (double)v[u].y; s0[2] += (double)v[u].z; s0[3] += (double)v[u].w;
+                    s1[0] += (double)v[u + 1].x; s1[1] += (double)v[u + 1].y; s1[2] += (double)v[u + 1].z; s1[3] += (double)v[u + 1].w;
+                }
+            }
+            for (; b + RD_FIN_Q < nblk; b += 2 * RD_FIN_Q) {
+                const float4 a = *reinterpret_cast<const float4*>(src + (size_t)b * stride);
+                const float4 c = *reinterpret_cast<const float4*>(src + (size_t)(b + RD_FIN_Q) * stride);
+                s0[0] += (double)a.x; s0[1] += (double)a.y; s0[2] += (double)a.z; s0[3] += (double)a.w;
+                s1[0] += (double)c.x; s1[1] += (double)c.y; s1[2] += (double)c.z; s1[3] += (double)c.w;
+            }
+            if (b < nblk) {
+                const float4 a = *reinterpret_cast<const float4*>(src + (size_t)b * stride);
+                s0[0] += (double)a.x; s0[1] += (double)a.y; s0[2] += (double)a.z; s0[3] += (double)a.w;
+            }
+        }
+    } else {
+        const long c = ((long)blockIdx.x - g_blocks) * RD_FIN_E + el;
+        if (c < Mg)
+            for (int b = q; b < nblk; b += RD_FIN_Q) s0[0] += part_cs[(size_t)b * MgPad + c];
+    }
+#pragma unroll
+    for (int j = 0; j < 4; ++j) red[q][el][j] = s0[j] + s1[j];
+    __syncthreads();
+    if (q == 0) {
+        double s[4];
+#pragma unroll
+        for (int j = 0; j < 4; ++j) {
+            s[j] = red[0][el][j];
+#pragma unroll
+            for (int i = 1; i < RD_FIN_Q; ++i) s[j] += red[i][el][j];
+        }
+        if (!is_cs) {
+            if (e < total) {
+                const int m = (int)(e / ng4), n0 = 4 * (int)(e - (long)m * ng4);
+#pragma unroll
+                for (int j = 0; j < 4; ++j) {
+                    if (n0 + j < Ng) {
+                        float* d = G + (size_t)m * ldg + n0 + j;
+                        *d = accumulate ? (*d + (float)s[j]) : (float)s[j];
+                    }
+                }
+            }
+        } else {
+            const long c = ((long)blockIdx.x - g_blocks) * RD_FIN_E + el;
+            if (c < Mg) colsum[c] = accumulate ? (colsum[c] + (float)s[0]) : (float)s[0];
+        }
+    }
+}
+
 const GpeRdSwitches& gpe_rd_switches()
 {
     static const GpeRdSwitches sw = {gpe_dbg_env("GPE_RD_DEEP", -1), gpe_dbg_env("GPE_RD_NOPC", 0)};
@@ -1236,6 +1309,13 @@
 
 static int rd_finish(const RdParams& p, const GpeRdPlan& plan, float* G, int ldG, float* colsum, int accumulate, hipStream_t s)
 {
+    if (plan.NgPad % 4 == 0 && !(((uintptr_t)p.part) & 15)) {
+        const long blocks4 = gpe_cdiv((long)p.Mg * ((p.Ng + 3) >> 2), RD_FIN_E) + (colsum ? gpe_cdiv(p.Mg, RD_FIN_E) : 0);
+        hipLaunchKernelGGL(gpe_redgemm_finish4, dim3(blocks4), dim3(RD_FIN_E * RD_FIN_Q), 0, s, p.part, p.part_cs, plan.nblk, p.Mg, p.Ng,
+                           plan.MgPad, plan.NgPad, G, ldG, colsum, accumulate);
+        GPE_CHECK_LAUNCH();
+        return GPE_OK;
+    }
     const long blocks = gpe_cdiv((long)p.Mg * p.Ng, RD_FIN_E) + (colsum ? gpe_cdiv(p.Mg, RD_FIN_E) : 0);
     hipLaunchKernelGGL(gpe_redgemm_finish, dim3(blocks), dim3(RD_FIN_E * RD_FIN_Q), 0, s, p.part, p.part_cs, plan.nblk, p.Mg, p.Ng,
                        plan.MgPad, plan.NgPad, G, ldG, colsum, accumulate);
diff --git a/garment-pattern-estimation_amd/ops.py b/garment-pattern-estimation_amd/ops.py
--- a/garment-pattern-estimation_amd/ops.py
+++ b/garment-pattern-estimation_amd/ops.py
@@ -10,7 +10,7 @@
 
 from . import _lib as L
 from . import streams
-from ._opbase import (F32, F64, _WS, _dev_check, _rows2d, _rows3d, _stitch_ldw, _ticket, _word, _workspace,
+from ._opbase import (F32, F64, _WS, _chain_tickets, _dev_check, _rows2d, _rows3d, _stitch_ldw, _ticket, _word, _workspace,
                       edge_workspace, f16x3_words, round_up)
 
 
@@ -370,6 +370,24 @@
     return coef, dg, db
 
 
+def point_sums_coef(g, ldg, mx, mn, ldagg, stats, rows, C, count, gamma, beta, training, bound=None):
+    dev = stats.device
+    psb = L.query('gpe_point_sums_blocks')
+    part = torch.empty(psb, 2, C, device=dev, dtype=torch.float64)
+    if not training:
+        L.call('gpe_edge_bwd_point_sums', g, ldg, mx, mn, ldagg, stats, rows, C, part, None if bound is None else bound[0])
+        coef, dg, db = bn_bwd_coef(part, psb, stats, C, count, gamma, beta, training)
+        if bound is not None:
+            L.call('gpe_edge_dz3_bound', bound[0], coef, C, bound[1], bound[2])
+        return coef, dg, db
+    coef, dg, db = torch.empty(4, C, device=dev, dtype=F32), _gbuf(gamma), _gbuf(beta)
+    chain = torch.empty(16, 2, C, device=dev, dtype=torch.float64)
+    sg, a3, out = bound if bound is not None else (None, None, None)
+    L.call('gpe_edge_bwd_point_sums_coef', g, ldg, mx, mn, ldagg, stats, rows, C, float(count), part, chain, coef, dg, db, sg, a3, out,
+           _chain_tickets(L.query('gpe_point_sums_coef_tickets', C), dev))
+    return coef, dg, db
+
+
 def bn_stats(blk, eps, training=False, momentum=None, part=None, nblk=0, count=0):
     if training:
         return bn_finalize(part, nblk, blk.W.shape[0], count, blk.gamma, blk.beta, eps, momentum, blk.running_mean, blk.running_var,
@@ -452,10 +470,10 @@
     else:
         edge_redgemm(u=dz, ldu=dz.stride(0), v=src, v_shift=st_prev[0], dims=dims, Mg=Cl, Ng=Cp, G=G, ldG=Cp, colsum=db, part=part,
                      amax_u=amax[0], amax_v=amax[1], ws=ws, lazy=lazy)
-    sums = torch.empty(1, 2, Cp, device=W.device, dtype=torch.float64)
-    dW = _gbuf(W)
-    L.call('gpe_bn_bwd_from_G', G, Cp, db, W, W.stride(0), Cl, Cp, st_prev, sums, dW, Cp)
-    coef_p, dgp, dbp = bn_bwd_coef(sums, 1, st_prev, Cp, count, gp, bp, training)
+    dW, dgp, dbp, coef_p = _gbuf(W), _gbuf(gp), _gbuf(bp), torch.empty(4, Cp, device=W.device, dtype=F32)
+    L.call('gpe_bn_bwd_from_G_coef', G, Cp, db, W, W.stride(0), Cl, Cp, st_prev, float(count), None, dW, Cp, coef_p, dgp, dbp)
+    if not training:
+        coef_p[1:3].zero_()
     filed[l, 'W'], filed[l, 'b'] = _gret(W, dW), _gret(b, db)
     filed[l - 1, 'gamma'], filed[l - 1, 'beta'] = _gret(gp, dgp), _gret(bp, dbp)
     (out, ldo), (dP, lddp) = ((src.t, src.ld), (None, 0)) if first is None else ((first[0], Cp), (first[1], first[1].stride(0)))
@@ -804,8 +822,6 @@
             with lane.fork([idx]):
                 rev = knn_reverse(idx)
 
-        psb = L.query('gpe_point_sums_blocks')
-        part = torch.empty(psb, 2, Fo, device=dev, dtype=torch.float64)
         g_last, be_last = blocks[-1].gamma, blocks[-1].beta
         a_last = acts[-1]
         lz = NO_LAZY
@@ -814,11 +830,9 @@
             lazy = a_last.dtype == torch.float16 and L.query('gpe_edge_lazy_dz3_ok', B, N, k, Fo, widths[-2]) == 1
             if a_last.dtype == torch.float16 and not lazy:
                 a_last = a_last.float()
-            L.call('gpe_edge_bwd_point_sums', g_out, ldg, mx, mn, ldF, stats[-1], BN, Fo, part,
-                   _word(words, 2 * nb) if lazy else None)
-            coef, dg, dbe = bn_bwd_coef(part, psb, stats[-1], Fo, E, g_last, be_last, training)
+            bound = (_word(words, 2 * nb), _word(words, nb - 1), _word(words, 2 * nb - 1)) if lazy else None
+            coef, dg, dbe = point_sums_coef(g_out, ldg, mx, mn, ldF, stats[-1], BN, Fo, E, g_last, be_last, training, bound)
             if lazy:
-                L.call('gpe_edge_dz3_bound', _word(words, 2 * nb), coef, Fo, _word(words, nb - 1), _word(words, 2 * nb - 1))
                 lz = (g_out, ldg, amx, amn, ldF, coef)
             else:
                 L.call('gpe_edge_dz3', a_last, ldF, g_out, ldg, amx, amn, ldF, coef, B, N, k, Fo, _word(words, 2 * nb - 1))
@@ -828,8 +842,7 @@
             if aggr == 'add':
                 gs = torch.empty(BN, Fo, device=dev, dtype=F32)
                 L.call('gpe_scale', g_out.contiguous(), float(k), gs, gs.numel())
-            L.call('gpe_edge_bwd_point_sums', gs, gs.stride(0), abar, abar, ldF, stats[-1], BN, Fo, part, None)
-            coef, dg, dbe = bn_bwd_coef(part, psb, stats[-1], Fo, E, g_last, be_last, training)
+            coef, dg, dbe = point_sums_coef(gs, gs.stride(0), abar, abar, ldF, stats[-1], BN, Fo, E, g_last, be_last, training)
             L.call('gpe_edge_dz3_all', a_last, ldF, g_out, ldg, 1.0 / k if aggr == 'mean' else 1.0, coef, B, N, k, Fo,
                    _word(words, 2 * nb - 1))
         filed[nb - 1, 'gamma'], filed[nb - 1, 'beta'] = _gret(g_last, dg), _gret(be_last, dbe)
@@ -1344,10 +1357,7 @@
         a, st = acts[-1], stats[-1]
         C = blocks[-1].W.shape[0]
         g_l, be_l = blocks[-1].gamma, blocks[-1].beta
-        psb = L.query('gpe_point_sums_blocks')
-        part = torch.empty(psb, 2, C, device=dev, dtype=torch.float64)
-        L.call('gpe_edge_bwd_point_sums', gy, C, a, a, a.stride(0), st, M, C, part, None)
-        coef, dgam, dbet = bn_bwd_coef(part, psb, st, C, M, g_l, be_l, training)
+        coef, dgam, dbet = point_sums_coef(gy, C, a, a, a.stride(0), st, M, C, M, g_l, be_l, training)
         words = ctx.words
         ews = edge_workspace(1, M, 1, 4, dev)
         L.call('gpe_edge_dz3_all', a, a.stride(0), gy, C, 1.0, coef, 1, M, 1, C, _word(words, 2 * n - 1))
diff --git a/include/gpe_hip_chain.h b/include/gpe_hip_chain.h
--- /dev/null
+++ b/include/gpe_hip_chain.h
@@ -0,0 +1,20 @@
+#ifndef GPE_HIP_CHAIN_H
+#define GPE_HIP_CHAIN_H
+#include <stdint.h>
+#ifdef __cplusplus
+extern "C" {
+#endif
+
+int gpe_bn_bwd_from_G_coef(const float* G, int ldG, const float* db, const float* w_next, int ldw, int Cn, int C, const float* stats,
+                           double count, double* sums, float* dw, int lddw, float* coef, float* dgamma, float* dbeta, void* stream);
+
+int gpe_point_sums_coef_tickets(int C);
+
+int gpe_edge_bwd_point_sums_coef(const float* g, int ldg, const float* mx, const float* mn, int ldagg, const float* stats, long rows,
+                                 int C, double count, double* part, double* chain_ws, float* coef, float* dgamma, float* dbeta,
+                                 uint32_t* amax_sg, const uint32_t* amax_a3, uint32_t* amax_out, uint32_t* tickets, void* stream);
+
+#ifdef __cplusplus
+}
+#endif
+#endif
```

Result: no change. 3835 garments/s, median of 6 (+0.7%).
